# xswang/xflow

Measured on NVIDIA H100. Metric: training examples/sec, higher is better.
Workload: dtype f32

## Files before the change

### xflow_b200/csrc/kernels.cu

```cuda
#include <cuda_runtime.h>
#include <stdint.h>
#include <stdlib.h>

#include "kernels.h"
#include "table.cuh"

__global__ void xf_k_fill(uint8_t* base, uint64_t cap, uint32_t stride, int lazy) {
  const uint64_t chunks_per_row = stride / 16;
  const uint64_t total = cap * chunks_per_row;
  for (uint64_t c = (uint64_t)blockIdx.x * blockDim.x + threadIdx.x; c < total;
       c += (uint64_t)gridDim.x * blockDim.x) {
    uint64_t r = c / chunks_per_row;
    uint32_t q = (uint32_t)(c % chunks_per_row);
    uint4 v = make_uint4(0, 0, 0, 0);
    if (q == 0) {
      v.x = 0xFFFFFFFFu; v.y = 0xFFFFFFFFu;
      if (!lazy) v.w = XF_NEG_ZERO_BITS;
    }
    *reinterpret_cast<uint4*>(base + r * stride + (uint64_t)q * 16) = v;
  }
}

template <int VEC>
__device__ __forceinline__ void xf_ldv(const float* p, float (&o)[VEC]) {
  if (VEC == 4) { float4 t = __ldcg(reinterpret_cast<const float4*>(p)); o[0] = t.x; o[1 % VEC] = t.y; o[2 % VEC] = t.z; o[3 % VEC] = t.w; }
  else if (VEC == 2) { float2 t = __ldcg(reinterpret_cast<const float2*>(p)); o[0] = t.x; o[1 % VEC] = t.y; }
  else { o[0] = __ldcg(p); }
}
template <int VEC>
__device__ __forceinline__ void xf_stv(float* p, const float (&o)[VEC]) {
  if (VEC == 4) *reinterpret_cast<float4*>(p) = make_float4(o[0], o[1 % VEC], o[2 % VEC], o[3 % VEC]);
  else if (VEC == 2) *reinterpret_cast<float2*>(p) = make_float2(o[0], o[1 % VEC]);
  else *p = o[0];
}
template <int VEC, bool SLOTG, bool STAMP>
__global__ void __launch_bounds__(256)
xf_k_update(XfTableView t, const uint32_t* __restrict__ slots, uint64_t n, int tps, double rows,
            const float* __restrict__ gw, const float* __restrict__ gv, int part,
            unsigned long long* __restrict__ live_total, const uint32_t* __restrict__ n_dev,
            const uint32_t* __restrict__ rows_dev, uint32_t extra_base, uint32_t extra_n,
            const float* __restrict__ v0_side, XfStampView sv) {
  __shared__ unsigned int s_live;
  if (threadIdx.x == 0) s_live = 0;
  __syncthreads();
  uint64_t n_head = n;
  if (n_dev != nullptr) {
    n_head = min((uint64_t)__ldg(n_dev), (uint64_t)extra_base);
    n = n_head + extra_n;
    rows = (double)__ldg(rows_dev);
  }
  unsigned int live_acc = 0;
  const int K = t.K;
  const unsigned lane = threadIdx.x & 31u;
  const uint64_t gwarp = ((uint64_t)blockIdx.x * blockDim.x + threadIdx.x) >> 5;
  const uint64_t nwarps = ((uint64_t)gridDim.x * blockDim.x) >> 5;
  const int q = (int)(lane & (unsigned)(tps - 1));
  const int gi = (int)(lane / (unsigned)tps);
  const int ngroups = 32 / tps;
  const int leader = (int)(lane & ~(unsigned)(tps - 1));
  const unsigned group_mask = (tps == 32) ? 0xffffffffu : (((1u << tps) - 1u) << leader);
  const int nchunk = K / VEC;

  for (uint64_t base = gwarp * 32; base < n; base += nwarps * 32) {
    const uint64_t e_fwd = base + lane;
    const uint64_t e_i = (SLOTG && e_fwd < n) ? (n - 1 - e_fwd) : e_fwd;
    const uint64_t e_phys = (e_i < n_head) ? e_i : (uint64_t)extra_base + (e_i - n_head);
    const uint32_t s_lane = (e_fwd < n) ? __ldcs(slots + e_phys) : 0xFFFFFFFFu;
    unsigned pend = __ballot_sync(0xffffffffu, s_lane != 0xFFFFFFFFu);
    if (live_total != nullptr && lane == 0) live_acc += __popc(pend);

    while (pend) {
      const int cnt = __popc(pend);
      const unsigned src = (gi < cnt) ? __fns(pend, 0, gi + 1) : 0u;
      const uint32_t s = __shfl_sync(0xffffffffu, s_lane, (int)src);
      const uint64_t i = __shfl_sync(0xffffffffu, (unsigned long long)e_i, (int)src);
      const uint64_t i_phys = __shfl_sync(0xffffffffu, (unsigned long long)e_phys, (int)src);
      uint8_t* rowp = (gi < cnt) ? xf_row(t, s) : nullptr;
      pend = (cnt <= ngroups) ? 0u : (pend & ~((2u << __fns(pend, 0, ngroups)) - 1u));

      const bool lat = K > 0 && (part & 2) && rowp != nullptr;
      float* vp = lat ? xf_row_v(rowp) : nullptr;
      float* nvp = lat ? xf_row_nv(rowp, K) : nullptr;
      float* zvp = lat ? xf_row_zv(rowp, K) : nullptr;
      float v0[VEC], n0[VEC], z0[VEC];
#pragma unroll
      for (int e = 0; e < VEC; ++e) { v0[e] = 0.f; n0[e] = 0.f; z0[e] = 0.f; }
      const bool has0 = lat && q < nchunk;
      if (has0) {
        xf_ldv<VEC>(vp + q * VEC, v0);
        if (t.opt == XF_OPT_FTRL) { xf_ldv<VEC>(nvp + q * VEC, n0); xf_ldv<VEC>(zvp + q * VEC, z0); }
      }
      float p0[VEC];
#pragma unroll
      for (int e = 0; e < VEC; ++e) p0[e] = 0.f;
      if (SLOTG && v0_side != nullptr && has0) {
        const uint64_t tok = (i_phys < (uint64_t)extra_base) ? i_phys : (uint64_t)__ldg(slots + i_phys + extra_n);
        xf_ldv<VEC>(v0_side + tok * (uint64_t)K + q * VEC, p0);
      }
      float ca0[VEC];
#pragma unroll
      for (int e = 0; e < VEC; ++e) ca0[e] = 0.f;
      if (SLOTG && t.canon && has0) xf_ldv<VEC>(xf_row_ca(t, rowp) + q * VEC, ca0);
      double accL = 0.0, accA = 0.0;
      if (SLOTG && has0) {
        const double2 a = __ldcg(reinterpret_cast<const double2*>(xf_row_acc(rowp, K)));
        accL = a.x;
        accA = a.y;
      }
      XfHead h;
      h.key = 0; h.flags = 0; h.w = h.n = h.z = 0.f; h.g = 0.0;
      if (q == 0 && rowp != nullptr) h = xf_load_head(rowp);
      const uint64_t key = __shfl_sync(group_mask, (unsigned long long)h.key, leader);
      const uint32_t flags = __shfl_sync(group_mask, h.flags, leader);
      if (rowp == nullptr) continue;

      if (q == 0) {
        if (!SLOTG) xf_apply_pending(t, h);
        if (part & 1) {
          const float g = SLOTG ? xf_div_rows((float)h.g, rows) : gw[i];
          xf_opt_coord(t, g, h.w, h.n, h.z);
        }
        if (SLOTG) h.g = -0.0;
        if (K > 0 && (part & 2)) h.flags |= XF_FLAG_V_READY;
        xf_store_head_t(t, rowp, h);
        if (STAMP) sv.stamp[s] = sv.now;
      }
      if (lat) {
        const bool ready = (flags & XF_FLAG_V_READY) != 0;
        for (int c = q; c < nchunk; c += tps) {
          const int k = c * VEC;
          float v[VEC], g[VEC], nn[VEC], zz[VEC];
#pragma unroll
          for (int e = 0; e < VEC; ++e) { v[e] = v0[e]; nn[e] = n0[e]; zz[e] = z0[e]; }
          if (c != q && ready) {
            xf_ldv<VEC>(vp + k, v);
            if (t.opt == XF_OPT_FTRL) { xf_ldv<VEC>(nvp + k, nn); xf_ldv<VEC>(zvp + k, zz); }
          }
          if (!ready) {
#pragma unroll
            for (int e = 0; e < VEC; ++e) { v[e] = xf_v_init(t, key, (uint32_t)(k + e)); nn[e] = 0.f; zz[e] = 0.f; }
          }
          if (SLOTG) {
            float vp0[VEC];
#pragma unroll
            for (int e = 0; e < VEC; ++e) vp0[e] = v[e];
            if (v0_side != nullptr) {
              if (c == q) {
#pragma unroll
                for (int e = 0; e < VEC; ++e) vp0[e] = p0[e];
              } else {
                const uint64_t tok = (i_phys < (uint64_t)extra_base) ? i_phys : (uint64_t)__ldg(slots + i_phys + extra_n);
                xf_ldv<VEC>(v0_side + tok * (uint64_t)K + k, vp0);
              }
            }
            if (t.canon) {
              float ca[VEC];
#pragma unroll
              for (int e = 0; e < VEC; ++e) ca[e] = ca0[e];
              if (c != q) xf_ldv<VEC>(xf_row_ca(t, rowp) + k, ca);
#pragma unroll
              for (int e = 0; e < VEC; ++e) g[e] = xf_div_rows((float)((double)ca[e] - (double)vp0[e] * accL), rows);
              const float zero[VEC] = {};
              xf_stv<VEC>(xf_row_ca(t, rowp) + k, zero);
            } else {
#pragma unroll
              for (int e = 0; e < VEC; ++e) g[e] = xf_div_rows((float)(accA - (double)vp0[e] * accL), rows);
            }
          } else {
#pragma unroll
            for (int e = 0; e < VEC; ++e) g[e] = gv[i * (uint64_t)K + k + e];
          }
          if (t.opt == XF_OPT_FTRL) {
#pragma unroll
            for (int e = 0; e < VEC; ++e) xf_ftrl_coord(t, g[e], v[e], nn[e], zz[e]);
            xf_stv<VEC>(nvp + k, nn);
            xf_stv<VEC>(zvp + k, zz);
          } else {
#pragma unroll
            for (int e = 0; e < VEC; ++e) xf_sgd_coord(t, g[e], v[e]);
          }
          xf_stv<VEC>(vp + k, v);
        }
        if (SLOTG) {
          __syncwarp(group_mask);
          if (q == 0) *reinterpret_cast<double2*>(xf_row_acc(rowp, K)) = make_double2(0.0, 0.0);
        }
      }
    }
  }
  if (live_total != nullptr) {
    if (lane == 0 && live_acc) atomicAdd(&s_live, live_acc);
    __syncthreads();
    if (threadIdx.x == 0 && s_live) atomicAdd_system(live_total, (unsigned long long)s_live);
  }
}

template <bool INSERT>
__global__ void xf_k_probe(XfTableView t, const uint64_t* __restrict__ keys, uint64_t n,
                           uint32_t* __restrict__ slots, float* __restrict__ w_out, XfStampView sv) {
  for (uint64_t i = (uint64_t)blockIdx.x * blockDim.x + threadIdx.x; i < n;
       i += (uint64_t)gridDim.x * blockDim.x) {
    XfHead h;
    h.w = 0.f;
    int64_t s = xf_probe<INSERT, true>(t, keys[i], &h, &sv);
    slots[i] = s >= 0 ? (uint32_t)s : 0xFFFFFFFFu;
    if (w_out) {
      if (s >= 0) xf_apply_pending(t, h);
      w_out[i] = s >= 0 ? h.w : 0.f;
    }
  }
}

__global__ void xf_k_gather_v(XfTableView t, const uint32_t* __restrict__ slots, const uint64_t* __restrict__ keys,
                              uint64_t n, float* __restrict__ v_out) {
  const int K = t.K;
  const uint64_t total = n * (uint64_t)K;
  for (uint64_t x = (uint64_t)blockIdx.x * blockDim.x + threadIdx.x; x < total;
       x += (uint64_t)gridDim.x * blockDim.x) {
    const uint64_t i = x / K;
    const int k = (int)(x % K);
    const uint32_t s = slots[i];
    float v = 0.f;
    if (s != 0xFFFFFFFFu) {
      const uint8_t* rowp = xf_row(t, s);
      const uint32_t flags = __ldcg(reinterpret_cast<const uint32_t*>(rowp + XF_OFF_FLAGS));
      v = (flags & XF_FLAG_V_READY) ? __ldcg(reinterpret_cast<const float*>(rowp + 32) + k)
                                    : xf_v_init(t, keys[i], (uint32_t)k);
    }
    v_out[x] = v;
  }
}

__global__ void xf_k_import(XfTableView t, const uint32_t* __restrict__ slots, uint64_t n,
                            const float* w, const float* nw, const float* zw, const float* v,
                            const float* nv, const float* zv) {
  const int K = t.K;
  const uint64_t per = (uint64_t)K + 1;
  const uint64_t total = n * per;
  for (uint64_t x = (uint64_t)blockIdx.x * blockDim.x + threadIdx.x; x < total;
       x += (uint64_t)gridDim.x * blockDim.x) {
    const uint64_t i = x / per;
    const int c = (int)(x % per);
    const uint32_t s = slots[i];
    if (s == 0xFFFFFFFFu) continue;
    uint8_t* rowp = xf_row(t, s);
    if (c == 0) {
      if (w) {
        if (t.lazy) {
          XfHead h;
          h.key = *reinterpret_cast<const uint64_t*>(rowp);
          h.w = w[i]; h.n = nw ? nw[i] : 0.f; h.z = zw ? zw[i] : 0.f; h.flags = 0u; h.g = 0.0;
          xf_lazy_store(t, rowp, h, true);
        } else {
          *reinterpret_cast<float2*>(rowp + XF_OFF_STATE) = make_float2(w[i], nw ? nw[i] : 0.f);
          *reinterpret_cast<float*>(rowp + XF_OFF_STATE + 8) = zw ? zw[i] : 0.f;
          *reinterpret_cast<unsigned long long*>(rowp + 8) = XF_NEG_ZERO_BITS64;
        }
      }
      if (v && K > 0) *reinterpret_cast<uint32_t*>(rowp + XF_OFF_FLAGS) = XF_FLAG_V_READY;
    } else if (v) {
      const int k = c - 1;
      xf_row_v(rowp)[k] = v[i * K + k];
      if (k == 0) *reinterpret_cast<double2*>(xf_row_acc(rowp, K)) = make_double2(0.0, 0.0);
      if (t.opt == XF_OPT_FTRL) {
        xf_row_nv(rowp, K)[k] = nv ? nv[i * K + k] : 0.f;
        xf_row_zv(rowp, K)[k] = zv ? zv[i * K + k] : 0.f;
      }
    }
  }
}

__global__ void xf_k_export(XfTableView t, const uint32_t* __restrict__ slots, const uint64_t* __restrict__ keys,
                            uint64_t n, float* w, float* nw, float* zw, float* v, float* nv, float* zv,
                            uint8_t* present) {
  const int K = t.K;
  const uint64_t per = (uint64_t)K + 1;
  const uint64_t total = n * per;
  for (uint64_t x = (uint64_t)blockIdx.x * blockDim.x + threadIdx.x; x < total;
       x += (uint64_t)gridDim.x * blockDim.x) {
    const uint64_t i = x / per;
    const int c = (int)(x % per);
    const uint32_t s = slots[i];
    const bool have = s != 0xFFFFFFFFu;
    const uint8_t* rowp = have ? xf_row(t, s) : nullptr;
    if (c == 0) {
      XfHead h;
      h.w = h.n = h.z = 0.f;
      if (have) {
        h = xf_load_head(rowp);
        xf_apply_pending(t, h);
      }
      if (present) present[i] = have ? 1 : 0;
      if (w) w[i] = h.w;
      if (nw) nw[i] = h.n;
      if (zw) zw[i] = h.z;
    } else if (v) {
      const int k = c - 1;
      float vv = 0.f, nn = 0.f, zz = 0.f;
      if (have) {
        const uint32_t flags = __ldcg(reinterpret_cast<const uint32_t*>(rowp + XF_OFF_FLAGS));
        if (flags & XF_FLAG_V_READY) {
          vv = __ldcg(reinterpret_cast<const float*>(rowp + 32) + k);
          if (t.opt == XF_OPT_FTRL) {
            nn = __ldcg(xf_row_nv(const_cast<uint8_t*>(rowp), K) + k);
            zz = __ldcg(xf_row_zv(const_cast<uint8_t*>(rowp), K) + k);
          }
        } else {
          vv = xf_v_init(t, keys[i], (uint32_t)k);
        }
      }
      v[i * K + k] = vv;
      if (nv) nv[i * K + k] = nn;
      if (zv) zv[i * K + k] = zz;
    }
  }
}

__global__ void xf_k_rehash(XfTableView src, XfTableView dst, XfKeep keep, const uint32_t* __restrict__ src_stamp,
                            uint32_t* __restrict__ dst_stamp) {
  const uint64_t cap = src.mask + 1;
  const uint32_t chunks = src.stride / 16;
  for (uint64_t r = (uint64_t)blockIdx.x * blockDim.x + threadIdx.x; r < cap;
       r += (uint64_t)gridDim.x * blockDim.x) {
    const uint8_t* srow = xf_row(src, r);
    uint4 a = *reinterpret_cast<const uint4*>(srow);
    uint64_t key = (uint64_t)a.x | ((uint64_t)a.y << 32);
    if (key == XF_EMPTY_KEY) continue;
    const uint32_t stamp = src_stamp != nullptr ? src_stamp[r] : 0u;
    if (src_stamp != nullptr && !xf_keeps(keep, stamp, key)) continue;
    XfHead h;
    int64_t s = xf_probe<true>(dst, key, &h);
    if (s < 0) continue;
    uint8_t* drow = xf_row(dst, (uint64_t)s);
    *reinterpret_cast<uint2*>(drow + 8) = make_uint2(a.z, a.w);
    for (uint32_t c = 1; c < chunks; ++c)
      *reinterpret_cast<uint4*>(drow + 16 * c) = *reinterpret_cast<const uint4*>(srow + 16 * c);
    if (dst_stamp != nullptr) dst_stamp[s] = stamp;
  }
}

__global__ void xf_k_list_keys(XfTableView t, uint64_t* keys_out, unsigned long long* count, uint64_t max_out) {
  const uint64_t cap = t.mask + 1;
  for (uint64_t r = (uint64_t)blockIdx.x * blockDim.x + threadIdx.x; r < cap;
       r += (uint64_t)gridDim.x * blockDim.x) {
    const uint64_t key = *reinterpret_cast<const uint64_t*>(xf_row(t, r));
    if (key == XF_EMPTY_KEY) continue;
    unsigned long long idx = atomicAdd(count, 1ull);
    if (idx < max_out) keys_out[idx] = key;
  }
}

static int g_sm_count = 0;
int xf_sms() {
  if (g_sm_count == 0) {
    int dev = 0;
    cudaGetDevice(&dev);
    cudaDeviceGetAttribute(&g_sm_count, cudaDevAttrMultiProcessorCount, dev);
    if (g_sm_count <= 0) g_sm_count = 132;
  }
  return g_sm_count;
}
int xf_grid_for(uint64_t work_items, int block, int blocks_per_sm) {
  uint64_t want = (work_items + block - 1) / block;
  uint64_t cap = (uint64_t)xf_sms() * blocks_per_sm;
  if (want < 1) want = 1;
  return (int)(want < cap ? want : cap);
}

int xf_vec_for(int K) { return K <= 0 ? 1 : (K % 4 == 0 ? 4 : (K % 2 == 0 ? 2 : 1)); }
int xf_tps_for(int K) {
  if (K <= 0) return 1;
  int chunks = K / xf_vec_for(K);
  int tps = 1;
  while (tps < chunks && tps < 32) tps <<= 1;
  return tps;
}

void xf_launch_fill(const XfTableView& t, cudaStream_t st) {
  uint64_t cap = t.mask + 1;
  uint64_t total = cap * (t.stride / 16);
  xf_k_fill<<<xf_grid_for(total, 256, 16), 256, 0, st>>>(t.base, cap, t.stride, t.lazy);
}

template <bool SLOTG, bool STAMP = false>
static void xf_launch_update_t(const XfTableView& t, const uint32_t* slots, uint64_t n, double rows,
                               const float* gw, const float* gv, int part, unsigned long long* live_total,
                               cudaStream_t st, const uint32_t* n_dev = nullptr, const uint32_t* rows_dev = nullptr,
                               uint32_t extra_base = 0, uint32_t extra_n = 0, const float* v0_side = nullptr,
                               XfStampView sv = XfStampView{nullptr, 0u}) {
  const int tps = xf_tps_for(t.K);
  const int grid = xf_grid_for(n * (uint64_t)tps, 256, 8);
#define XF_UPD_ARGS t, slots, n, tps, rows, gw, gv, part, live_total, n_dev, rows_dev, extra_base, extra_n, v0_side, sv
  switch (xf_vec_for(t.K)) {
    case 4: xf_k_update<4, SLOTG, STAMP><<<grid, 256, 0, st>>>(XF_UPD_ARGS); break;
    case 2: xf_k_update<2, SLOTG, STAMP><<<grid, 256, 0, st>>>(XF_UPD_ARGS); break;
    default: xf_k_update<1, SLOTG, STAMP><<<grid, 256, 0, st>>>(XF_UPD_ARGS); break;
  }
#undef XF_UPD_ARGS
}

void xf_launch_update_touched_dev(const XfTableView& t, const uint32_t* touched, uint64_t work_bound,
                                  const uint32_t* n_dev, const uint32_t* rows_dev, uint32_t extra_base,
                                  uint32_t extra_n, const float* v0_side, unsigned long long* unique_total,
                                  cudaStream_t st) {
  xf_launch_update_t<true>(t, touched, work_bound + extra_n, 1.0, nullptr, nullptr, 3, unique_total, st, n_dev, rows_dev,
                           extra_base, extra_n, v0_side);
}

__global__ void xf_k_flush_pending(XfTableView t) {
  const uint64_t cap = t.mask + 1;
  for (uint64_t r = (uint64_t)blockIdx.x * blockDim.x + threadIdx.x; r < cap; r += (uint64_t)gridDim.x * blockDim.x) {
    uint8_t* rowp = xf_row(t, r);
    XfHead h = xf_load_head(rowp);
    if (h.key == XF_EMPTY_KEY || !xf_lazy_has_pending(h)) continue;
    xf_apply_pending(t, h);
    xf_lazy_store(t, rowp, h);
  }
}
void xf_launch_flush_pending(const XfTableView& t, cudaStream_t st) {
  xf_k_flush_pending<<<xf_grid_for(t.mask + 1, 256, 8), 256, 0, st>>>(t);
}

void xf_launch_update_touched(const XfTableView& t, const uint32_t* touched, uint64_t nnz, double rows,
                              unsigned long long* unique_total, const XfStampView& sv, cudaStream_t st) {
  if (nnz == 0) return;
  if (sv.stamp)
    xf_launch_update_t<true, true>(t, touched, nnz, rows, nullptr, nullptr, 3, unique_total, st, nullptr, nullptr, 0, 0,
                                   nullptr, sv);
  else
    xf_launch_update_t<true>(t, touched, nnz, rows, nullptr, nullptr, 3, unique_total, st);
}

void xf_launch_update_pushed(const XfTableView& t, const uint32_t* slots, uint64_t n, const float* gw,
                             const float* gv, cudaStream_t st) {
  if (n == 0) return;
  int part = (gw ? 1 : 0) | (gv ? 2 : 0);
  xf_launch_update_t<false>(t, slots, n, 1.0, gw, gv, part, nullptr, st);
}

void xf_launch_probe(const XfTableView& t, const uint64_t* keys, uint64_t n, bool insert, uint32_t* slots,
                     float* w_out, cudaStream_t st, const XfStampView& sv) {
  if (n == 0) return;
  const int grid = xf_grid_for(n, 256, 8);
  if (insert) xf_k_probe<true><<<grid, 256, 0, st>>>(t, keys, n, slots, w_out, sv);
  else xf_k_probe<false><<<grid, 256, 0, st>>>(t, keys, n, slots, w_out, sv);
}

void xf_launch_gather_v(const XfTableView& t, const uint32_t* slots, const uint64_t* keys, uint64_t n,
                        float* v_out, cudaStream_t st) {
  if (n == 0 || t.K == 0) return;
  xf_k_gather_v<<<xf_grid_for(n * t.K, 256, 8), 256, 0, st>>>(t, slots, keys, n, v_out);
}

void xf_launch_import(const XfTableView& t, const uint32_t* slots, uint64_t n, const float* w, const float* nw,
                      const float* zw, const float* v, const float* nv, const float* zv, cudaStream_t st) {
  if (n == 0) return;
  xf_k_import<<<xf_grid_for(n * (t.K + 1), 256, 8), 256, 0, st>>>(t, slots, n, w, nw, zw, v, nv, zv);
}

void xf_launch_export(const XfTableView& t, const uint32_t* slots, const uint64_t* keys, uint64_t n, float* w,
                      float* nw, float* zw, float* v, float* nv, float* zv, uint8_t* present, cudaStream_t st) {
  if (n == 0) return;
  xf_k_export<<<xf_grid_for(n * (t.K + 1), 256, 8), 256, 0, st>>>(t, slots, keys, n, w, nw, zw, v, nv, zv, present);
}

void xf_launch_rehash(const XfTableView& src, const XfTableView& dst, const XfKeep& keep, const uint32_t* src_stamp,
                      uint32_t* dst_stamp, cudaStream_t st) {
  xf_k_rehash<<<xf_grid_for(src.mask + 1, 256, 8), 256, 0, st>>>(src, dst, keep, src_stamp, dst_stamp);
}

void xf_launch_list_keys(const XfTableView& t, uint64_t* keys_out, unsigned long long* count, uint64_t max_out,
                         cudaStream_t st) {
  xf_k_list_keys<<<xf_grid_for(t.mask + 1, 256, 8), 256, 0, st>>>(t, keys_out, count, max_out);
}
```

### xflow_b200/csrc/mg_kernels.cu

```cuda
#include <cuda_runtime.h>
#include <stdint.h>

#include "kernels.h"
#include "mg.cuh"
#include "table.cuh"

#define XF_NO_SLOT 0xFFFFFFFFu

__device__ __forceinline__ unsigned long long xf_globaltimer() {
  unsigned long long t;
  asm volatile("mov.u64 %0, %%globaltimer;" : "=l"(t));
  return t;
}
__device__ __forceinline__ uint64_t xf_ld_acquire_sys(const uint64_t* p) {
  uint64_t v;
  asm volatile("ld.acquire.sys.global.u64 %0, [%1];" : "=l"(v) : "l"(p) : "memory");
  return v;
}
__device__ __forceinline__ void xf_st_release_sys(uint64_t* p, uint64_t v) {
  asm volatile("st.release.sys.global.u64 [%0], %1;" ::"l"(p), "l"(v) : "memory");
}

__global__ void xf_k_signal(XfPeers peers, XfSlabLayout L, int S, int me, int flag, uint64_t step, int parity,
                            const uint32_t* __restrict__ bucket_cnt, uint32_t rows) {
  const int q = threadIdx.x;
  if (q >= S) return;
  uint8_t* slab = peers.slab[q];
  if (bucket_cnt != nullptr) {
    volatile uint32_t* m = reinterpret_cast<uint32_t*>(slab + L.off_meta) + ((size_t)(parity * XF_MG_MAX_SHARDS + me) * 4);
    m[0] = bucket_cnt[q];
    m[1] = rows;
  }
  xf_st_release_sys(reinterpret_cast<uint64_t*>(slab + L.off_flags) + (size_t)flag * XF_MG_MAX_SHARDS + me, step);
}

__global__ void xf_k_wait(const uint64_t* __restrict__ flags, int S, uint64_t step, int* error,
                          unsigned long long timeout_ns) {
  const int q = threadIdx.x;
  if (q >= S) return;
  const unsigned long long t0 = xf_globaltimer();
  while (xf_ld_acquire_sys(flags + q) < step) {
    if (xf_globaltimer() - t0 > timeout_ns) {
      *error = 4;
      break;
    }
    __nanosleep(64);
  }
}

#define XF_RT_THREADS 512
#define XF_RT_TOK 4
#define XF_RT_TILE (XF_RT_THREADS * XF_RT_TOK)

__device__ __forceinline__ int xf_dev_shard_of(uint64_t key, uint64_t width, int S) {
  const uint64_t s = key / width;
  return (int)(s < (uint64_t)S ? s : (uint64_t)S - 1);
}

__device__ __forceinline__ uint32_t xf_row_of(const uint32_t* a, uint32_t lo, uint32_t hi, uint32_t j) {
  while (lo < hi) {
    const uint32_t mid = (lo + hi + 1) >> 1;
    if (a[mid] <= j) lo = mid; else hi = mid - 1;
  }
  return lo;
}

__global__ void __launch_bounds__(XF_RT_THREADS)
xf_k_route(const uint32_t* __restrict__ row_ptr, const uint64_t* __restrict__ keys, uint32_t rows, uint64_t width,
           int S, int me, uint32_t cap, XfPeers peers, uint64_t off_keys, uint64_t off_rows,
           uint32_t* __restrict__ bucket_cnt, uint32_t* __restrict__ tok_pos) {
  __shared__ uint64_t s_key[XF_RT_TILE];
  __shared__ uint32_t s_row[XF_RT_TILE];
  __shared__ uint32_t s_rp[XF_RT_TILE + 1];
  __shared__ uint32_t s_cnt[XF_MG_MAX_SHARDS], s_base[XF_MG_MAX_SHARDS], s_off[XF_MG_MAX_SHARDS + 1];
  __shared__ uint32_t s_rlo, s_rhi;
  const uint32_t beg = __ldg(row_ptr), end = __ldg(row_ptr + rows);
  const uint32_t j0 = beg + blockIdx.x * XF_RT_TILE;
  if (j0 >= end) return;
  const uint32_t j1 = min(j0 + (uint32_t)XF_RT_TILE, end);
  if (threadIdx.x < XF_MG_MAX_SHARDS) s_cnt[threadIdx.x] = 0;
  if (threadIdx.x == 0) s_rlo = xf_row_of(row_ptr, 0, rows - 1, j0);
  if (threadIdx.x == 32) s_rhi = xf_row_of(row_ptr, 0, rows - 1, j1 - 1);
  __syncthreads();
  const uint32_t rlo = s_rlo, rhi = s_rhi;
  const bool cached = (rhi - rlo + 1) <= (uint32_t)XF_RT_TILE;
  if (cached)
    for (uint32_t r = threadIdx.x; r <= rhi - rlo + 1; r += XF_RT_THREADS) s_rp[r] = __ldg(row_ptr + rlo + r);
  __syncthreads();

  uint64_t my_key[XF_RT_TOK];
  uint32_t my_rank[XF_RT_TOK], my_row[XF_RT_TOK];
  int my_q[XF_RT_TOK];
#pragma unroll
  for (int i = 0; i < XF_RT_TOK; ++i) {
    const uint32_t j = j0 + threadIdx.x + i * XF_RT_THREADS;
    my_q[i] = -1;
    if (j < j1) {
      my_key[i] = __ldcs(keys + j);
      my_q[i] = xf_dev_shard_of(my_key[i], width, S);
      my_rank[i] = atomicAdd(&s_cnt[my_q[i]], 1u);
      my_row[i] = cached ? (rlo + xf_row_of(s_rp, 0, rhi - rlo, j)) : xf_row_of(row_ptr, rlo, rhi, j);
    }
  }
  __syncthreads();
  if (threadIdx.x < S && s_cnt[threadIdx.x]) s_base[threadIdx.x] = atomicAdd(bucket_cnt + threadIdx.x, s_cnt[threadIdx.x]);
  if (threadIdx.x == 0) {
    uint32_t o = 0;
    for (int q = 0; q < S; ++q) { s_off[q] = o; o += s_cnt[q]; }
    s_off[S] = o;
  }
  __syncthreads();
#pragma unroll
  for (int i = 0; i < XF_RT_TOK; ++i) {
    if (my_q[i] < 0) continue;
    const uint32_t j = j0 + threadIdx.x + i * XF_RT_THREADS;
    const uint32_t at = s_off[my_q[i]] + my_rank[i];
    s_key[at] = my_key[i];
    s_row[at] = my_row[i];
    tok_pos[j] = (uint32_t)my_q[i] * cap + s_base[my_q[i]] + my_rank[i];
  }
  __syncthreads();
  const uint32_t n = j1 - j0;
  for (uint32_t x = threadIdx.x; x < n; x += XF_RT_THREADS) {
    int q = 0;
    while (x >= s_off[q + 1]) ++q;
    const uint64_t dst = (uint64_t)me * cap + s_base[q] + (x - s_off[q]);
    reinterpret_cast<uint64_t*>(peers.slab[q] + off_keys)[dst] = s_key[x];
    reinterpret_cast<uint32_t*>(peers.slab[q] + off_rows)[dst] = s_row[x];
  }
}

template <bool FM, int VEC>
__global__ void __launch_bounds__(256)
xf_k_pull_tokens(XfTableView t, const uint64_t* __restrict__ in_keys, const uint32_t* __restrict__ meta, int S, int me,
                 uint32_t cap, XfPeers peers, uint64_t off_vals, uint32_t* __restrict__ slots,
                 float* __restrict__ side_v, uint4* __restrict__ stash) {
  __shared__ uint32_t s_pre[XF_MG_MAX_SHARDS + 1];
  if (threadIdx.x == 0) {
    uint32_t o = 0;
    for (int s = 0; s < S; ++s) { s_pre[s] = o; o += min(meta[s * 4], cap); }
    s_pre[S] = o;
  }
  __syncthreads();
  const uint32_t total = s_pre[S];
  const int K = t.K;
  for (uint32_t x = blockIdx.x * blockDim.x + threadIdx.x; x < total; x += gridDim.x * blockDim.x) {
    int s = 0;
    while (x >= s_pre[s + 1]) ++s;
    const uint32_t i = x - s_pre[s];
    const uint64_t key = __ldcs(in_keys + (uint64_t)s * cap + i);
    const uint64_t home = xf_home_slot(t, key);
    XfHead h = FM ? xf_load_head_l1(xf_row(t, home)) : xf_load_head(xf_row(t, home));
    const int64_t r = xf_probe_from<true>(t, key, home, h);
    float w = 0.f, st = 0.f, qt = 0.f;
    if (!FM && stash != nullptr) {
      const uint64_t q1 = xf_raw_q1(h), q2 = xf_raw_q2(h);
      uint64_t q3 = xf_raw_q3(h);
      if ((uint32_t)(q1 >> 32) == xf_lazy_check(q2)) q3 |= XF_TAG_MASK;
      __stcs(stash + ((uint64_t)s * cap + i), make_uint4((uint32_t)q2, (uint32_t)(q2 >> 32), (uint32_t)q3, (uint32_t)(q3 >> 32)));
    }
    if (r >= 0) {
      xf_apply_pending(t, h);
      w = h.w;
      if (FM) {
        float* sv = (s > 0 && side_v != nullptr) ? side_v + ((uint64_t)s * cap + i) * (uint64_t)K : nullptr;
        if ((h.flags & XF_FLAG_V_READY) && (K & 7) == 0) {
          const float* vp = reinterpret_cast<const float*>(xf_row(t, (uint64_t)r) + 32);
          for (int k = 0; k < K; k += 8) {
            float v[8];
            xf_ld8_l1(vp + k, v);
#pragma unroll
            for (int e = 0; e < 8; ++e) { st += v[e]; qt = __fadd_rn(qt, __fmul_rn(v[e], v[e])); }
            if (sv) {
              __stcs(reinterpret_cast<float4*>(sv + k), make_float4(v[0], v[1], v[2], v[3]));
              __stcs(reinterpret_cast<float4*>(sv + k + 4), make_float4(v[4], v[5], v[6], v[7]));
            }
          }
        } else if (h.flags & XF_FLAG_V_READY) {
          const float* vp = reinterpret_cast<const float*>(xf_row(t, (uint64_t)r) + 32);
          for (int k = 0; k < K; k += VEC) {
            float v[VEC];
            if (VEC == 4) { const float4 q4 = __ldca(reinterpret_cast<const float4*>(vp + k)); v[0] = q4.x; v[1 % VEC] = q4.y; v[2 % VEC] = q4.z; v[3 % VEC] = q4.w; }
            else if (VEC == 2) { const float2 q2 = __ldca(reinterpret_cast<const float2*>(vp + k)); v[0] = q2.x; v[1 % VEC] = q2.y; }
            else { v[0] = __ldca(vp + k); }
#pragma unroll
            for (int e = 0; e < VEC; ++e) { st += v[e]; qt = __fadd_rn(qt, __fmul_rn(v[e], v[e])); }
            if (sv) {
              if (VEC == 4) __stcs(reinterpret_cast<float4*>(sv + k), make_float4(v[0], v[1 % VEC], v[2 % VEC], v[3 % VEC]));
              else if (VEC == 2) __stcs(reinterpret_cast<float2*>(sv + k), make_float2(v[0], v[1 % VEC]));
              else __stcs(sv + k, v[0]);
            }
          }
        } else {
          for (int k = 0; k < K; ++k) {
            const float v = xf_v_init(t, key, (uint32_t)k);
            st += v;
            qt = __fadd_rn(qt, __fmul_rn(v, v));
            if (sv) __stcs(sv + k, v);
          }
        }
      }
    }
    slots[(uint64_t)s * cap + i] = r >= 0 ? (uint32_t)r : XF_NO_SLOT;
    const uint64_t dst = (uint64_t)me * cap + i;
    if (FM) reinterpret_cast<float4*>(peers.slab[s] + off_vals)[dst] = make_float4(w, st, qt, 0.f);
    else reinterpret_cast<float*>(peers.slab[s] + off_vals)[dst] = w;
  }
}

template <bool FM>
__global__ void __launch_bounds__(256)
xf_k_rows(const uint32_t* __restrict__ row_ptr, const uint8_t* __restrict__ labels, int B, int mode,
          const uint32_t* __restrict__ tok_pos, const void* __restrict__ vals, float* __restrict__ rowv,
          float* __restrict__ loss_out, float* __restrict__ pctr_out, float* __restrict__ abs_loss_sum) {
  __shared__ float s_abs[8];
  float abs_acc = 0.f;
  const int lane = threadIdx.x & 31;
  const int wpb = blockDim.x >> 5;
  const int gwarp = blockIdx.x * wpb + (threadIdx.x >> 5);
  const int nwarps = gridDim.x * wpb;
  for (int row = gwarp; row < B; row += nwarps) {
    const uint32_t beg = __ldg(row_ptr + row), end = __ldg(row_ptr + row + 1);
    float wsum = 0.f, ssum = 0.f, qsum = 0.f;
    for (uint32_t j = beg + lane; j < end; j += 32) {
      const uint32_t pos = __ldcs(tok_pos + j);
      if (FM) {
        const float4 a = __ldcg(reinterpret_cast<const float4*>(vals) + pos);
        wsum += a.x; ssum += a.y; qsum += a.z;
      } else {
        wsum += __ldcg(reinterpret_cast<const float*>(vals) + pos);
      }
    }
    const float wx = xf_warp_sum(wsum);
    float Ssum = 0.f, arg = wx;
    if (FM) {
      Ssum = xf_warp_sum(ssum);
      const float Q = xf_warp_sum(qsum);
      arg = __fadd_rn(wx, __fsub_rn(__fmul_rn(Ssum, Ssum), Q));
    }
    const float pctr = xf_sigmoid(arg);
    if (mode == 1) {
      if (lane == 0 && pctr_out) pctr_out[row] = pctr;
      continue;
    }
    const float loss = __fsub_rn(pctr, (float)labels[row]);
    if (lane == 0) {
      if (loss_out) loss_out[row] = loss;
      if (FM) reinterpret_cast<float2*>(rowv)[row] = make_float2(loss, Ssum);
      else rowv[row] = loss;
    }
    abs_acc += fabsf(loss);
  }
  if (abs_loss_sum != nullptr && mode == 0) {
    if (lane == 0) s_abs[threadIdx.x >> 5] = abs_acc;
    __syncthreads();
    if (threadIdx.x == 0) {
      float tot = 0.f;
      for (int w = 0; w < wpb; ++w) tot += s_abs[w];
      atomicAdd(abs_loss_sum, tot);
    }
  }
}

__global__ void xf_k_bcast_rowv(const uint32_t* __restrict__ src, uint32_t n_words, XfPeers peers, uint64_t off_rowv,
                                uint64_t dst_word_off) {
  uint32_t* dst = reinterpret_cast<uint32_t*>(peers.slab[blockIdx.y] + off_rowv) + dst_word_off;
  for (uint32_t x = blockIdx.x * blockDim.x + threadIdx.x; x < n_words; x += gridDim.x * blockDim.x) dst[x] = __ldcg(src + x);
}

__global__ void __launch_bounds__(256)
xf_k_push_tokens_lr(XfTableView t, const uint32_t* __restrict__ slots, const uint32_t* __restrict__ in_rows,
                    const float* __restrict__ rowv, const uint32_t* __restrict__ meta_s, uint32_t cap, uint32_t seq,
                    uint64_t* rows_by_seq, unsigned long long* uniq_remote, const uint4* __restrict__ stash) {
  __shared__ unsigned int s_open;
  if (threadIdx.x == 0) s_open = 0;
  const uint32_t n = min(__ldg(meta_s), cap);
  const int fs = xf_fix_shift(n);
  if (blockIdx.x == 0 && threadIdx.x == 0)
    rows_by_seq[seq] = (uint64_t)__ldg(meta_s + 1) | ((uint64_t)fs << 32);
  __syncthreads();
  unsigned int open_acc = 0;
  const int lane = threadIdx.x & 31;
  const uint32_t wpb = blockDim.x >> 5;
  const uint32_t gwarp = blockIdx.x * wpb + (threadIdx.x >> 5);
  const uint32_t nwarps = gridDim.x * wpb;
  uint32_t s_n[2], r_n[2];
  uint4 b_n[2];
#define XF_PUSH_FETCH(base_)                                                        \
  _Pragma("unroll") for (int u = 0; u < 2; ++u) {                                    \
    const uint32_t i = (base_) + 32u * u + lane;                                     \
    s_n[u] = XF_NO_SLOT; r_n[u] = 0u; b_n[u] = make_uint4(0u, 0u, 0u, 0u);            \
    if (i < n) {                                                                     \
      s_n[u] = __ldcs(slots + i);                                                    \
      r_n[u] = __ldcs(in_rows + i);                                                  \
      b_n[u] = __ldcs(stash + (uint64_t)i);                                          \
    }                                                                                \
  }
  uint32_t base = gwarp * 64;
  if (base < n) { XF_PUSH_FETCH(base) }
  for (; base < n; base += nwarps * 64) {
    uint32_t s[2];
    float l[2];
    uint64_t q2[2], q3[2];
#pragma unroll
    for (int u = 0; u < 2; ++u) {
      s[u] = s_n[u];
      l[u] = 0.f;
      q2[u] = 0ull; q3[u] = (uint64_t)seq;
      if (s[u] == XF_NO_SLOT) continue;
      l[u] = __ldcg(rowv + r_n[u]);
      q2[u] = (uint64_t)b_n[u].x | ((uint64_t)b_n[u].y << 32);
      q3[u] = (uint64_t)b_n[u].z | ((uint64_t)b_n[u].w << 32);
    }
    if (base + nwarps * 64 < n) { XF_PUSH_FETCH(base + nwarps * 64) }
    bool lead[2], issued[2], reload[2];
    long long fix[2];
    uint64_t q2n[2], o2[2], o3[2];
#pragma unroll
    for (int u = 0; u < 2; ++u) {
      const bool valid = s[u] != XF_NO_SLOT;
      const unsigned grp = __match_any_sync(0xffffffffu, valid ? s[u] : (0xFFFFFF00u | (uint32_t)lane));
      lead[u] = valid && lane == __ffs(grp) - 1;
      fix[u] = valid ? xf_fix_of(l[u], fs) : 0ll;
      if (__any_sync(0xffffffffu, valid && __popc(grp) > 1)) {
        long long sum = 0ll;
        for (int b = 0; b < 32; ++b) {
          const long long o = __shfl_sync(0xffffffffu, fix[u], b);
          if ((grp >> b) & 1u) sum += o;
        }
        fix[u] = sum;
      }
      issued[u] = false;
      q2n[u] = q2[u]; o2[u] = q2[u]; o3[u] = q3[u];
      reload[u] = lead[u] && (q3[u] & XF_TAG_MASK) == XF_TAG_MASK;
      if (lead[u] && !reload[u]) {
        xf_lazy_fold(t, 0ull, q2[u], q3[u], seq, q2n[u]);
        issued[u] = xf_lazy_deposit_issue(xf_row(t, s[u]), q2[u], q3[u], q2n[u], seq, fix[u], o2[u], o3[u]);
      }
    }
#pragma unroll
    for (int u = 0; u < 2; ++u) {
      if (!lead[u]) continue;
      uint8_t* rowp = xf_row(t, s[u]);
      bool stale = false;
      if (!reload[u] &&
          xf_lazy_deposit_resolve(rowp, issued[u], q2[u], q3[u], o2[u], o3[u], seq, fix[u], &stale))
        ++open_acc;
      if (stale) {
        uint64_t r2n;
        xf_lazy_fold(t, 0ull, o2[u], o3[u], seq, r2n);
        if (xf_lazy_deposit(t, rowp, o2[u], o3[u], r2n, seq, fix[u])) ++open_acc;
      } else if (reload[u]) {
        const XfHead h = xf_load_head(rowp);
        uint64_t r2n;
        xf_lazy_fold(t, xf_raw_q1(h), xf_raw_q2(h), xf_raw_q3(h), seq, r2n);
        if (xf_lazy_deposit(t, rowp, xf_raw_q2(h), xf_raw_q3(h), r2n, seq, fix[u])) ++open_acc;
      }
    }
  }
#undef XF_PUSH_FETCH
  if (open_acc) atomicAdd(&s_open, open_acc);
  __syncthreads();
  if (threadIdx.x == 0 && s_open && uniq_remote) atomicAdd_system(uniq_remote, (unsigned long long)s_open);
}

template <bool FM>
__global__ void __launch_bounds__(256)
xf_k_acc_tokens(XfTableView t, const uint32_t* __restrict__ slots, const uint32_t* __restrict__ in_rows,
                const void* __restrict__ rowv, const uint32_t* __restrict__ meta_s, uint32_t cap,
                uint32_t* __restrict__ touched, int log2nc) {
  extern __shared__ __align__(16) unsigned char xf_smem[];
  const int K = t.K;
  const int NC = (FM && log2nc >= 0) ? (1 << log2nc) : 0;
  double* c_acc = reinterpret_cast<double*>(xf_smem);
  uint32_t* c_tag = reinterpret_cast<uint32_t*>(xf_smem + (size_t)NC * 24);
  uint32_t* c_tok = c_tag + NC;
  if (NC) {
    for (int e = threadIdx.x; e < NC; e += blockDim.x) { c_tag[e] = XF_NO_SLOT; c_tok[e] = 0; }
    for (int e = threadIdx.x; e < NC * 3; e += blockDim.x) c_acc[e] = 0.0;
    __syncthreads();
  }
  const uint32_t n = min(__ldg(meta_s), cap);
  const int lane = threadIdx.x & 31;
  const uint32_t wpb = blockDim.x >> 5;
  const uint32_t gwarp = blockIdx.x * wpb + (threadIdx.x >> 5);
  const uint32_t nwarps = gridDim.x * wpb;
  for (uint32_t base = gwarp * 32; base < n; base += nwarps * 32) {
    const uint32_t i = base + lane;
    uint32_t s = XF_NO_SLOT;
    float loss = 0.f, Srow = 0.f;
    if (i < n) {
      s = __ldcs(slots + i);
      const uint32_t row = __ldcs(in_rows + i);
      if (FM) { const float2 a = __ldcg(reinterpret_cast<const float2*>(rowv) + row); loss = a.x; Srow = a.y; }
      else loss = __ldcg(reinterpret_cast<const float*>(rowv) + row);
    }
    const bool valid = s != XF_NO_SLOT;
    float gw_c = loss;
    if (FM) {
      gw_c = 0.f;
      for (int k = 0; k < K; ++k) gw_c += loss;
    }
    double gd = (double)gw_c, ld = (double)loss, ad = (double)loss * (double)Srow;
    const unsigned grp = __match_any_sync(0xffffffffu, valid ? s : (0xFFFFFF00u | (uint32_t)lane));
    const bool lead = valid && lane == __ffs(grp) - 1;
    if (__any_sync(0xffffffffu, valid && __popc(grp) > 1)) {
      double sg = 0.0, sl = 0.0, sa = 0.0;
      for (int b = 0; b < 32; ++b) {
        const double og = __shfl_sync(0xffffffffu, gd, b), ol = __shfl_sync(0xffffffffu, ld, b),
                     oa = __shfl_sync(0xffffffffu, ad, b);
        if ((grp >> b) & 1u) { sg += og; sl += ol; sa += oa; }
      }
      gd = sg; ld = sl; ad = sa;
    }
    bool first = false;
    if (lead) {
      bool cached = false;
      if (NC) {
        const uint32_t e = (s * 2654435761u) >> (32 - log2nc);
        const uint32_t prev = atomicCAS(c_tag + e, XF_NO_SLOT, s);
        if (prev == XF_NO_SLOT || prev == s) {
          cached = true;
          if (prev == XF_NO_SLOT) c_tok[e] = i;
          atomicAdd(c_acc + 3 * e, gd);
          atomicAdd(c_acc + 3 * e + 1, ld);
          atomicAdd(c_acc + 3 * e + 2, ad);
        }
      }
      if (!cached) {
        uint8_t* rowp = xf_row(t, s);
        const double old = atomicAdd(xf_row_g(rowp), gd);
        if (FM) { double* a = xf_row_acc(rowp, K); atomicAdd(a, ld); atomicAdd(a + 1, ad); }
        first = (unsigned long long)__double_as_longlong(old) == XF_NEG_ZERO_BITS64;
      }
    }
    if (i < n) __stcs(touched + i, first ? s : XF_NO_SLOT);
  }
  if (NC) {
    __syncthreads();
    for (int e = threadIdx.x; e < NC; e += blockDim.x) {
      const uint32_t s = c_tag[e];
      uint32_t rec = XF_NO_SLOT;
      if (s != XF_NO_SLOT) {
        uint8_t* rowp = xf_row(t, s);
        const double old = atomicAdd(xf_row_g(rowp), c_acc[3 * e]);
        if ((unsigned long long)__double_as_longlong(old) == XF_NEG_ZERO_BITS64) rec = s;
        double* a = xf_row_acc(rowp, K);
        atomicAdd(a, c_acc[3 * e + 1]);
        atomicAdd(a + 1, c_acc[3 * e + 2]);
      }
      touched[cap + (uint32_t)blockIdx.x * (uint32_t)NC + (uint32_t)e] = rec;
      touched[cap + (gridDim.x + (uint32_t)blockIdx.x) * (uint32_t)NC + (uint32_t)e] = c_tok[e];
    }
  }
}

int xf_step_cache_log2(int K);

void xf_launch_signal(const XfPeers& peers, const XfSlabLayout& L, int S, int me, int flag, uint64_t step, int parity,
                      const uint32_t* bucket_cnt, uint32_t rows, cudaStream_t st) {
  xf_k_signal<<<1, 32, 0, st>>>(peers, L, S, me, flag, step, parity, bucket_cnt, rows);
}
void xf_launch_wait(const uint64_t* flags, int S, uint64_t step, int* error, unsigned long long timeout_ns,
                    cudaStream_t st) {
  xf_k_wait<<<1, 32, 0, st>>>(flags, S, step, error, timeout_ns);
}
void xf_launch_route(const uint32_t* row_ptr, const uint64_t* keys, uint32_t rows, uint32_t nnz_bound, uint64_t width,
                     int S, int me, uint32_t cap, const XfPeers& peers, uint64_t off_keys, uint64_t off_rows,
                     uint32_t* bucket_cnt, uint32_t* tok_pos, cudaStream_t st) {
  if (rows == 0 || nnz_bound == 0) return;
  const uint32_t grid = (nnz_bound + XF_RT_TILE - 1) / XF_RT_TILE;
  xf_k_route<<<grid, XF_RT_THREADS, 0, st>>>(row_ptr, keys, rows, width, S, me, cap, peers, off_keys, off_rows,
                                              bucket_cnt, tok_pos);
}
void xf_launch_pull_tokens(const XfTableView& t, const uint64_t* in_keys, const uint32_t* meta, int S, int me,
                           uint32_t cap, uint64_t work_bound, const XfPeers& peers, uint64_t off_vals,
                           uint32_t* slots, float* side_v, void* stash, cudaStream_t st) {
  const int grid = xf_grid_for(work_bound ? work_bound : 1, 256, 8);
#define XF_PT_ARGS t, in_keys, meta, S, me, cap, peers, off_vals, slots, side_v, reinterpret_cast<uint4*>(stash)
  if (t.K == 0) {
    xf_k_pull_tokens<false, 1><<<grid, 256, 0, st>>>(XF_PT_ARGS);
  } else {
    switch (xf_vec_for(t.K)) {
      case 4: xf_k_pull_tokens<true, 4><<<grid, 256, 0, st>>>(XF_PT_ARGS); break;
      case 2: xf_k_pull_tokens<true, 2><<<grid, 256, 0, st>>>(XF_PT_ARGS); break;
      default: xf_k_pull_tokens<true, 1><<<grid, 256, 0, st>>>(XF_PT_ARGS); break;
    }
  }
#undef XF_PT_ARGS
}
void xf_launch_rows(bool fm, const uint32_t* row_ptr, const uint8_t* labels, int B, int mode, const uint32_t* tok_pos,
                    const void* vals, float* rowv, float* loss_out, float* pctr_out, float* abs_loss_sum,
                    cudaStream_t st) {
  if (B <= 0) return;
  const int grid = xf_grid_for((uint64_t)B * 32, 256, 8);
  if (fm) xf_k_rows<true><<<grid, 256, 0, st>>>(row_ptr, labels, B, mode, tok_pos, vals, rowv, loss_out, pctr_out, abs_loss_sum);
  else xf_k_rows<false><<<grid, 256, 0, st>>>(row_ptr, labels, B, mode, tok_pos, vals, rowv, loss_out, pctr_out, abs_loss_sum);
}
void xf_launch_bcast_rowv(const float* src, uint32_t n_words, int S, const XfPeers& peers, uint64_t off_rowv,
                          uint64_t dst_word_off, cudaStream_t st) {
  if (n_words == 0) return;
  dim3 grid((unsigned)xf_grid_for(n_words, 256, 1), (unsigned)S);
  if (grid.x > 64) grid.x = 64;
  xf_k_bcast_rowv<<<grid, 256, 0, st>>>(reinterpret_cast<const uint32_t*>(src), n_words, peers, off_rowv, dst_word_off);
}
void xf_launch_push_tokens_lr(const XfTableView& t, const uint32_t* slots, const uint32_t* in_rows, const float* rowv,
                              const uint32_t* meta_s, uint32_t cap, uint64_t work_bound, uint32_t seq,
                              uint64_t* rows_by_seq, unsigned long long* uniq_remote, const void* stash,
                              cudaStream_t st) {
  const int grid = xf_grid_for(work_bound ? work_bound : 1, 256, 8);
  xf_k_push_tokens_lr<<<grid, 256, 0, st>>>(t, slots, in_rows, rowv, meta_s, cap, seq, rows_by_seq, uniq_remote,
                                             reinterpret_cast<const uint4*>(stash));
}
uint32_t xf_acc_touched_extra(int K, uint64_t work_bound) {
  const int lg = xf_step_cache_log2(K);
  if (lg < 0) return 0;
  return (uint32_t)xf_grid_for(work_bound ? work_bound : 1, 256, 8) << lg;
}
void xf_launch_acc_tokens(const XfTableView& t, const uint32_t* slots, const uint32_t* in_rows, const void* rowv,
                          const uint32_t* meta_s, uint32_t cap, uint64_t work_bound, uint32_t* touched,
                          cudaStream_t st) {
  const int grid = xf_grid_for(work_bound ? work_bound : 1, 256, 8);
  const int lg = xf_step_cache_log2(t.K);
  const size_t smem = lg >= 0 ? ((size_t)1 << lg) * 32 : 0;
  if (t.K > 0) xf_k_acc_tokens<true><<<grid, 256, smem, st>>>(t, slots, in_rows, rowv, meta_s, cap, touched, lg);
  else xf_k_acc_tokens<false><<<grid, 256, 0, st>>>(t, slots, in_rows, rowv, meta_s, cap, touched, -1);
}
```

### xflow_b200/csrc/step.cu

```cuda
#include <cuda_runtime.h>
#include <stdint.h>
#include <stdlib.h>

#include "kernels.h"
#include "table.cuh"

#define XF_NO_SLOT 0xFFFFFFFFu
#define XF_CACHED_CHUNKS 2

template <int VEC>
__device__ __forceinline__ void xf_ldv_step(const float* p, float (&o)[VEC]) {
  if (VEC == 4) { float4 t = __ldca(reinterpret_cast<const float4*>(p)); o[0] = t.x; o[1 % VEC] = t.y; o[2 % VEC] = t.z; o[3 % VEC] = t.w; }
  else if (VEC == 2) { float2 t = __ldca(reinterpret_cast<const float2*>(p)); o[0] = t.x; o[1 % VEC] = t.y; }
  else { o[0] = __ldca(p); }
}
template <int VEC>
__device__ __forceinline__ void xf_fm_token(const XfTableView& t, uint32_t slot, uint32_t flags, uint64_t key,
                                            float& st, float& qt) {
  const int K = t.K;
  st = 0.f;
  qt = 0.f;
  if ((flags & XF_FLAG_V_READY) && (K & 7) == 0) {
    const float* vp = reinterpret_cast<const float*>(xf_row(t, slot) + 32);
    for (int k = 0; k < K; k += 8) {
      float v[8];
      xf_ld8_l1(vp + k, v);
#pragma unroll
      for (int e = 0; e < 8; ++e) { st += v[e]; qt = __fadd_rn(qt, __fmul_rn(v[e], v[e])); }
    }
  } else if (flags & XF_FLAG_V_READY) {
    const float* vp = reinterpret_cast<const float*>(xf_row(t, slot) + 32);
    for (int k = 0; k < K; k += VEC) {
      float v[VEC];
      xf_ldv_step<VEC>(vp + k, v);
#pragma unroll
      for (int e = 0; e < VEC; ++e) { st += v[e]; qt = __fadd_rn(qt, __fmul_rn(v[e], v[e])); }
    }
  } else {
    for (int k = 0; k < K; ++k) {
      const float v = xf_v_init(t, key, (uint32_t)k);
      st += v;
      qt = __fadd_rn(qt, __fmul_rn(v, v));
    }
  }
}

template <bool FM, int VEC, bool ADMIT, bool STAMP, bool WEIGHT>
__global__ void __launch_bounds__(256)
xf_k_step(XfTableView t, const uint32_t* __restrict__ row_ptr, const uint64_t* __restrict__ keys,
          const uint8_t* __restrict__ labels, int B, int mode, uint32_t* __restrict__ touched,
          float* __restrict__ loss_out, float* __restrict__ pctr_out, float* __restrict__ abs_loss_sum,
          int log2nc, uint32_t touched_base, XfAdmitView adm, XfStampView sv, XfWeightView wv) {
  __shared__ float s_abs[8];
  extern __shared__ __align__(16) unsigned char xf_smem[];
  float abs_acc = 0.f;
  const int lane = threadIdx.x & 31;
  const int warps_per_block = blockDim.x >> 5;
  const int gwarp = blockIdx.x * warps_per_block + (threadIdx.x >> 5);
  const int nwarps = gridDim.x * warps_per_block;
  const int K = t.K;
  const int NC = (FM && log2nc >= 0) ? (1 << log2nc) : 0;
  double* c_acc = reinterpret_cast<double*>(xf_smem);
  uint32_t* c_tag = reinterpret_cast<uint32_t*>(xf_smem + (size_t)NC * 24);
  if (NC) {
    for (int e = threadIdx.x; e < NC; e += blockDim.x) c_tag[e] = XF_NO_SLOT;
    for (int e = threadIdx.x; e < NC * 3; e += blockDim.x) c_acc[e] = 0.0;
    __syncthreads();
  }

  for (int row = gwarp; row < B; row += nwarps) {
    const uint32_t beg = __ldg(row_ptr + row);
    const uint32_t end = __ldg(row_ptr + row + 1);
    if (WEIGHT && __ldg(wv.e + row) == 0.f) {
      if (lane == 0 && loss_out) loss_out[row] = 0.f;
      for (uint32_t j = beg + (uint32_t)lane; j < end; j += 32u) __stcs(touched + j, XF_NO_SLOT);
      continue;
    }
    const int chunks = (int)((end - beg + 63u) >> 6);

    float wsum = 0.f, ssum = 0.f, qsum = 0.f;
    uint32_t slot_c[2 * XF_CACHED_CHUNKS];
#pragma unroll
    for (int c = 0; c < 2 * XF_CACHED_CHUNKS; ++c) slot_c[c] = XF_NO_SLOT;

    for (int ch = 0; ch < chunks; ++ch) {
      const uint32_t j0 = beg + (uint32_t)ch * 64u + (uint32_t)lane;
      const uint32_t j1 = j0 + 32u;
      const bool v0 = j0 < end, v1 = j1 < end;
      const uint64_t k0 = v0 ? __ldcs(keys + j0) : 0ull;
      const uint64_t k1 = v1 ? __ldcs(keys + j1) : 0ull;
      const uint64_t p0 = xf_home_slot(t, k0), p1 = xf_home_slot(t, k1);
      XfHead h0, h1;
      h0.key = h1.key = XF_EMPTY_KEY;
      if (v0) h0 = FM ? xf_load_head_l1(xf_row(t, p0)) : xf_load_head(xf_row(t, p0));
      if (v1) h1 = FM ? xf_load_head_l1(xf_row(t, p1)) : xf_load_head(xf_row(t, p1));
      uint32_t s0 = XF_NO_SLOT, s1 = XF_NO_SLOT;
      bool r0 = false, r1 = false;
      if (v0) {
        const int64_t r = xf_probe_from<true, ADMIT, STAMP>(t, k0, p0, h0, &adm, &r0, &sv);
        if (r >= 0) { s0 = (uint32_t)r; wsum += h0.w; }
      }
      if (v1) {
        const int64_t r = xf_probe_from<true, ADMIT, STAMP>(t, k1, p1, h1, &adm, &r1, &sv);
        if (r >= 0) { s1 = (uint32_t)r; wsum += h1.w; }
      }
      if (ADMIT) xf_admit_append(adm, r0, k0, r1, k1);
      if (FM) {
        float st, qt;
        if (s0 != XF_NO_SLOT) { xf_fm_token<VEC>(t, s0, h0.flags, k0, st, qt); ssum += st; qsum += qt; }
        if (s1 != XF_NO_SLOT) { xf_fm_token<VEC>(t, s1, h1.flags, k1, st, qt); ssum += st; qsum += qt; }
      }
#pragma unroll
      for (int c = 0; c < XF_CACHED_CHUNKS; ++c)
        if (ch == c) { slot_c[2 * c] = s0; slot_c[2 * c + 1] = s1; }
    }

    const float wx = xf_warp_sum(wsum);
    float S = 0.f, arg = wx;
    if (FM) {
      S = xf_warp_sum(ssum);
      const float Q = xf_warp_sum(qsum);
      const float v_y = __fsub_rn(__fmul_rn(S, S), Q);
      arg = __fadd_rn(wx, v_y);
    }
    const float pctr = xf_sigmoid(arg);
    if (mode == 1) {
      if (lane == 0 && pctr_out) pctr_out[row] = pctr;
      continue;
    }
    float loss = __fsub_rn(pctr, (float)labels[row]);
    if (lane == 0 && loss_out) loss_out[row] = loss;
    if (WEIGHT) loss = __fmul_rn(__ldg(wv.e + row), loss);
    abs_acc += fabsf(loss);

    float gw_c = loss;
    if (FM) {
      gw_c = 0.f;
      for (int k = 0; k < K; ++k) gw_c += loss;
    }
    const double gw_d = (double)gw_c;
    for (int ch = 0; ch < chunks; ++ch) {
      const uint32_t j0 = beg + (uint32_t)ch * 64u + (uint32_t)lane;
      const uint32_t j1 = j0 + 32u;
      uint32_t s0 = XF_NO_SLOT, s1 = XF_NO_SLOT;
      if (ch < XF_CACHED_CHUNKS) {
#pragma unroll
        for (int c = 0; c < XF_CACHED_CHUNKS; ++c)
          if (ch == c) { s0 = slot_c[2 * c]; s1 = slot_c[2 * c + 1]; }
      } else {
        XfHead h;
        if (j0 < end) { const int64_t r = xf_probe<false>(t, __ldg(keys + j0), &h); if (r >= 0) s0 = (uint32_t)r; }
        if (j1 < end) { const int64_t r = xf_probe<false>(t, __ldg(keys + j1), &h); if (r >= 0) s1 = (uint32_t)r; }
      }
      const unsigned g0 = __match_any_sync(0xffffffffu, (s0 != XF_NO_SLOT) ? s0 : (0xFFFFFF00u | (uint32_t)lane));
      const unsigned g1 = __match_any_sync(0xffffffffu, (s1 != XF_NO_SLOT) ? s1 : (0xFFFFFF00u | (uint32_t)lane));
      const bool lead0 = s0 != XF_NO_SLOT && lane == __ffs(g0) - 1;
      const bool lead1 = s1 != XF_NO_SLOT && lane == __ffs(g1) - 1;
      const double c0 = (double)__popc(g0), c1 = (double)__popc(g1);
      const double ld = (double)loss, ad = (double)loss * (double)S;
      double old0 = 0.0, old1 = 0.0;
      bool cached0 = false, cached1 = false;
      if (NC) {
        if (lead0) {
          const uint32_t e = (s0 * 2654435761u) >> (32 - log2nc);
          const uint32_t prev = atomicCAS(c_tag + e, XF_NO_SLOT, s0);
          if (prev == XF_NO_SLOT || prev == s0) {
            cached0 = true;
            atomicAdd(c_acc + 3 * e, gw_d * c0);
            atomicAdd(c_acc + 3 * e + 1, ld * c0);
            atomicAdd(c_acc + 3 * e + 2, ad * c0);
          }
        }
        if (lead1) {
          const uint32_t e = (s1 * 2654435761u) >> (32 - log2nc);
          const uint32_t prev = atomicCAS(c_tag + e, XF_NO_SLOT, s1);
          if (prev == XF_NO_SLOT || prev == s1) {
            cached1 = true;
            atomicAdd(c_acc + 3 * e, gw_d * c1);
            atomicAdd(c_acc + 3 * e + 1, ld * c1);
            atomicAdd(c_acc + 3 * e + 2, ad * c1);
          }
        }
      }
      if (lead0 && !cached0) old0 = atomicAdd(xf_row_g(xf_row(t, s0)), gw_d * c0);
      if (lead1 && !cached1) old1 = atomicAdd(xf_row_g(xf_row(t, s1)), gw_d * c1);
      if (FM) {
        if (lead0 && !cached0) { double* a = xf_row_acc(xf_row(t, s0), K); atomicAdd(a, ld * c0); atomicAdd(a + 1, ad * c0); }
        if (lead1 && !cached1) { double* a = xf_row_acc(xf_row(t, s1), K); atomicAdd(a, ld * c1); atomicAdd(a + 1, ad * c1); }
      }
      const bool f0 = lead0 && !cached0 && (unsigned long long)__double_as_longlong(old0) == XF_NEG_ZERO_BITS64;
      const bool f1 = lead1 && !cached1 && (unsigned long long)__double_as_longlong(old1) == XF_NEG_ZERO_BITS64;
      if (j0 < end) __stcs(touched + j0, f0 ? s0 : XF_NO_SLOT);
      if (j1 < end) __stcs(touched + j1, f1 ? s1 : XF_NO_SLOT);
    }
  }
  if (NC && mode == 0) {
    __syncthreads();
    for (int e = threadIdx.x; e < NC; e += blockDim.x) {
      const uint32_t s = c_tag[e];
      uint32_t rec = XF_NO_SLOT;
      if (s != XF_NO_SLOT) {
        uint8_t* rowp = xf_row(t, s);
        const double old = atomicAdd(xf_row_g(rowp), c_acc[3 * e]);
        if ((unsigned long long)__double_as_longlong(old) == XF_NEG_ZERO_BITS64) rec = s;
        double* a = xf_row_acc(rowp, K);
        atomicAdd(a, c_acc[3 * e + 1]);
        atomicAdd(a + 1, c_acc[3 * e + 2]);
      }
      touched[touched_base + (uint32_t)blockIdx.x * (uint32_t)NC + (uint32_t)e] = rec;
    }
  }
  if (abs_loss_sum != nullptr && mode == 0) {
    if (lane == 0) s_abs[threadIdx.x >> 5] = abs_acc;
    __syncthreads();
    if (threadIdx.x == 0) {
      float tot = 0.f;
      for (int w = 0; w < (int)(blockDim.x >> 5); ++w) tot += s_abs[w];
      atomicAdd(abs_loss_sum, tot);
    }
  }
}

int xf_sms();
int xf_grid_for(uint64_t work_items, int block, int blocks_per_sm);

#define XF_STEP_CACHE_LOG2 9
int xf_step_cache_log2(int K) {
  if (K <= 0) return -1;
  static const int lg = [] {
    const char* e = getenv("XFLOW_FM_CACHE_LOG2");
    const int v = (e && *e) ? atoi(e) : XF_STEP_CACHE_LOG2;
    return v < 0 ? 0 : (v > 10 ? 10 : v);
  }();
  return lg;
}
uint32_t xf_step_touched_extra(int K, int B) {
  const int lg = xf_step_cache_log2(K);
  if (lg < 0) return 0;
  return (uint32_t)xf_grid_for((uint64_t)B * 32, 256, 8) << lg;
}

void xf_launch_step(const XfTableView& t, const uint32_t* row_ptr, const uint64_t* keys, const uint8_t* labels,
                    int B, int mode, uint32_t* touched, uint32_t nnz, float* loss_out, float* pctr_out,
                    float* abs_loss_sum, const XfAdmitView* adm, const XfStampView& sv, const XfWeightView& wv,
                    cudaStream_t st) {
  if (B <= 0) return;
  const int block = 256;
  const int grid = xf_grid_for((uint64_t)B * 32, block, 8);
  const int lg = xf_step_cache_log2(t.K);
  const size_t smem = lg >= 0 ? ((size_t)1 << lg) * 28 : 0;
#define XF_STEP_ARGS t, row_ptr, keys, labels, B, mode, touched, loss_out, pctr_out, abs_loss_sum, lg, nnz, a, sv, wv
#define XF_STEP_LAUNCH_W(A, S, W)                                                             \
  if (t.K == 0) {                                                                             \
    xf_k_step<false, 1, A, S, W><<<grid, block, 0, st>>>(XF_STEP_ARGS);                       \
  } else {                                                                                    \
    switch (xf_vec_for(t.K)) {                                                                \
      case 4: xf_k_step<true, 4, A, S, W><<<grid, block, smem, st>>>(XF_STEP_ARGS); break;    \
      case 2: xf_k_step<true, 2, A, S, W><<<grid, block, smem, st>>>(XF_STEP_ARGS); break;    \
      default: xf_k_step<true, 1, A, S, W><<<grid, block, smem, st>>>(XF_STEP_ARGS); break;   \
    }                                                                                         \
  }
#define XF_STEP_LAUNCH(A, S)        \
  if (wv.e) {                       \
    XF_STEP_LAUNCH_W(A, S, true)    \
  } else {                          \
    XF_STEP_LAUNCH_W(A, S, false)   \
  }
  const XfAdmitView a = adm ? *adm : XfAdmitView{};
  const bool stamp = sv.stamp != nullptr;
  if (adm && stamp) {
    XF_STEP_LAUNCH(true, true)
  } else if (adm) {
    XF_STEP_LAUNCH(true, false)
  } else if (stamp) {
    XF_STEP_LAUNCH(false, true)
  } else {
    XF_STEP_LAUNCH(false, false)
  }
#undef XF_STEP_LAUNCH
#undef XF_STEP_LAUNCH_W
#undef XF_STEP_ARGS
}
```

### xflow_b200/csrc/table.cuh

```cuda
#pragma once
#include <cuda_runtime.h>
#include <stdint.h>

#define XF_EMPTY_KEY 0xFFFFFFFFFFFFFFFFull
#define XF_FLAG_V_READY 1u
#define XF_NEG_ZERO_BITS 0x80000000u
#define XF_NEG_ZERO_BITS64 0x8000000000000000ull
#define XF_MAX_PROBE 8192

enum { XF_OPT_FTRL = 0, XF_OPT_SGD = 1 };
enum { XF_INIT_DEFAULT = 0, XF_INIT_COUNTER = 1, XF_INIT_ZERO = 3 };

struct XfTableView {
  uint8_t* base;
  uint64_t mask;
  uint32_t log2cap;
  uint32_t bshift;
  uint32_t stride;
  int K;
  int opt;
  int v_init;
  float v_const;
  uint64_t seed;
  float alpha, beta, lambda1, lambda2, learning_rate;
  unsigned long long* size;
  int* error;
  int lazy;
  const uint64_t* rows_by_seq;
  int canon;
};
#define XF_ADM_POISSON 1
#define XF_ADM_BLOOM 2
#define XF_ADM_NEVER 3
#define XF_ADM_MAX_HASHES 8
struct XfAdmitView {
  int mode;
  uint32_t p24;
  uint64_t batch_mix;
  uint32_t threshold, log2_cells, hashes;
  uint64_t seed;
  const uint8_t* cells;
  unsigned long long* rej_n;
  uint64_t* rej_keys;
  unsigned long long* admitted;
};
struct XfKeep {
  uint32_t cutoff;
  int bounded;
  uint32_t s_star;
  uint64_t k_star;
};
struct XfStampView {
  uint32_t* stamp;
  uint32_t now;
};
struct XfWeightView {
  const float* e;
  const unsigned long long* W;
};
__host__ __device__ __forceinline__ bool xf_keeps(const XfKeep& k, uint32_t stamp, uint64_t key) {
  return stamp >= k.cutoff && (!k.bounded || stamp > k.s_star || (stamp == k.s_star && key <= k.k_star));
}
#define XF_TAG_LOCKED 0xFFFFFFFFu
#define XF_FIX_MAX_SHIFT 27
#define XF_TAG_MASK 0xFFFFull

__host__ __device__ inline int xf_fix_shift(uint64_t nnz) {
  int bits = 0;
  while (bits < 64 && (nnz >> bits) != 0ull) ++bits;
  const int s = 47 - bits;
  return s > XF_FIX_MAX_SHIFT ? XF_FIX_MAX_SHIFT : (s < 0 ? 0 : s);
}

__host__ __device__ inline uint32_t xf_acc_off(int K) { return (32u + 4u * (uint32_t)K + 15u) & ~15u; }
__host__ __device__ inline uint32_t xf_ca_off(int K, int opt) {
  return xf_acc_off(K) + 16u + ((opt == XF_OPT_FTRL) ? 8u * (uint32_t)K : 0u);
}
__host__ __device__ inline uint32_t xf_row_stride(int K, int opt, int canon = 0) {
  if (K <= 0) return 32u;
  uint32_t bytes = xf_ca_off(K, opt) + (canon ? 4u * (uint32_t)K : 0u);
  return (bytes + 31u) & ~31u;
}

#ifdef __CUDACC__

__device__ __forceinline__ uint64_t xf_probe_slot(const XfTableView& t, uint64_t key, uint32_t i) {
  const uint64_t m = key * 0x9E3779B97F4A7C15ull;
  const uint32_t bs = t.bshift;
  const uint64_t hb = m >> (64 - (t.log2cap - bs));
  const uint32_t b1 = (1u << bs) - 1u;
  const uint32_t j0 = (uint32_t)(m >> 9) & b1;
  const uint32_t k = i >> bs;
  const uint32_t j = (k == 0) ? ((j0 + i) & b1) : (i & b1);
  return (((hb + k) << bs) | j) & t.mask;
}
__device__ __forceinline__ uint64_t xf_home_slot(const XfTableView& t, uint64_t key) { return xf_probe_slot(t, key, 0); }

__host__ __device__ __forceinline__ uint64_t xf_splitmix64(uint64_t x) {
  x += 0x9E3779B97F4A7C15ull;
  x = (x ^ (x >> 30)) * 0xBF58476D1CE4E5B9ull;
  x = (x ^ (x >> 27)) * 0x94D049BB133111EBull;
  return x ^ (x >> 31);
}
__host__ __device__ __forceinline__ uint64_t xf_admit_cell(uint64_t key, uint64_t seed, uint32_t j, uint32_t log2_cells) {
  return xf_splitmix64(key ^ xf_splitmix64(seed + (uint64_t)(j + 1) * 0x9E3779B97F4A7C15ull)) >> (64 - log2_cells);
}
__device__ __forceinline__ bool xf_admit(const XfAdmitView& a, uint64_t key) {
  if (a.mode == XF_ADM_POISSON) return (uint32_t)(xf_splitmix64(key ^ a.batch_mix) >> 40) < a.p24;
  if (a.mode != XF_ADM_BLOOM) return false;
  uint32_t m = 255u;
  for (uint32_t j = 0; j < a.hashes; ++j) m = min(m, (uint32_t)__ldcg(a.cells + xf_admit_cell(key, a.seed, j, a.log2_cells)));
  return m >= a.threshold;
}
__device__ __forceinline__ void xf_admit_append(const XfAdmitView& a, bool r0, uint64_t k0, bool r1, uint64_t k1) {
  const unsigned m0 = __ballot_sync(0xffffffffu, r0), m1 = __ballot_sync(0xffffffffu, r1);
  if ((m0 | m1) == 0u) return;
  const unsigned lane = threadIdx.x & 31u;
  unsigned long long base = 0ull;
  if (lane == 0u) base = atomicAdd(a.rej_n, (unsigned long long)(__popc(m0) + __popc(m1)));
  base = __shfl_sync(0xffffffffu, base, 0);
  if (a.rej_keys) {
    const unsigned lt = (1u << lane) - 1u;
    if (r0) a.rej_keys[base + __popc(m0 & lt)] = k0;
    if (r1) a.rej_keys[base + __popc(m0) + __popc(m1 & lt)] = k1;
  }
}

__device__ __forceinline__ float xf_counter_normal(uint64_t key, uint32_t k, uint64_t seed) {
  uint64_t base = xf_splitmix64(key ^ xf_splitmix64(seed + 0x632BE59BD9B4E019ull * (uint64_t)(k + 1)));
  uint32_t sum = 0;
#pragma unroll
  for (int r = 0; r < 3; ++r) {
    uint64_t x = xf_splitmix64(base + (uint64_t)r);
    sum += (uint32_t)(x & 0xFFFF) + (uint32_t)((x >> 16) & 0xFFFF) + (uint32_t)((x >> 32) & 0xFFFF) +
           (uint32_t)((x >> 48) & 0xFFFF);
  }
  float u = __fmul_rn((float)((int32_t)sum - 6 * 65535), 1.0f / 65536.0f);
  return __fmul_rn(u, 1e-2f);
}
__device__ __forceinline__ float xf_v_init(const XfTableView& t, uint64_t key, uint32_t k) {
  if (t.v_init == XF_INIT_COUNTER) return xf_counter_normal(key, k, t.seed);
  if (t.v_init == XF_INIT_ZERO) return 0.0f;
  return t.v_const;
}

__device__ __forceinline__ uint8_t* xf_row(const XfTableView& t, uint64_t slot) {
  return t.base + slot * (uint64_t)t.stride;
}
__device__ __forceinline__ double* xf_row_g(uint8_t* row) { return reinterpret_cast<double*>(row + 8); }
#define XF_OFF_STATE 16
#define XF_OFF_FLAGS 28
__device__ __forceinline__ float* xf_row_v(uint8_t* row) { return reinterpret_cast<float*>(row + 32); }
__device__ __forceinline__ double* xf_row_acc(uint8_t* row, int K) { return reinterpret_cast<double*>(row + xf_acc_off(K)); }
__device__ __forceinline__ float* xf_row_nv(uint8_t* row, int K) { return reinterpret_cast<float*>(row + xf_acc_off(K) + 16); }
__device__ __forceinline__ float* xf_row_zv(uint8_t* row, int K) { return xf_row_nv(row, K) + K; }
__device__ __forceinline__ float* xf_row_ca(const XfTableView& t, uint8_t* row) { return reinterpret_cast<float*>(row + xf_ca_off(t.K, t.opt)); }

struct XfHead {
  uint64_t key;
  uint32_t flags;
  float w, n, z;
  double g;
};

__device__ __forceinline__ void xf_ld32_cg(const void* p, uint64_t& q0, uint64_t& q1, uint64_t& q2, uint64_t& q3) {
  asm volatile("ld.global.cg.v2.u64 {%0,%1}, [%4];\n\tld.global.cg.v2.u64 {%2,%3}, [%4+16];"
               : "=l"(q0), "=l"(q1), "=l"(q2), "=l"(q3) : "l"(p));
}
__device__ __forceinline__ void xf_ld32_ca(const void* p, uint64_t& q0, uint64_t& q1, uint64_t& q2, uint64_t& q3) {
  asm volatile("ld.global.ca.v2.u64 {%0,%1}, [%4];\n\tld.global.ca.v2.u64 {%2,%3}, [%4+16];"
               : "=l"(q0), "=l"(q1), "=l"(q2), "=l"(q3) : "l"(p));
}
__device__ __forceinline__ void xf_ld32_pair(const uint8_t* mine, uint64_t& q0, uint64_t& q1, uint64_t& q2, uint64_t& q3) {
  const uint32_t odd = threadIdx.x & 1u;
  const uint8_t* other = (const uint8_t*)__shfl_xor_sync(0xffffffffu, (unsigned long long)mine, 1);
  const uint8_t* r0 = odd ? other : mine;
  const uint8_t* r1 = odd ? mine : other;
  uint64_t x0 = 0, x1 = 0, y0 = 0, y1 = 0;
  asm volatile("{\n .reg .pred p0, p1;\n setp.ne.u64 p0, %4, 0;\n setp.ne.u64 p1, %5, 0;\n"
               " @p0 ld.global.cg.v2.u64 {%0,%1}, [%6];\n @p1 ld.global.cg.v2.u64 {%2,%3}, [%7];\n}"
               : "+l"(x0), "+l"(x1), "+l"(y0), "+l"(y1)
               : "l"(r0), "l"(r1), "l"(r0 + 16 * odd), "l"(r1 + 16 * odd));
  const uint64_t m0 = odd ? y0 : x0, m1 = odd ? y1 : x1;
  const uint64_t t0 = __shfl_xor_sync(0xffffffffu, odd ? x0 : y0, 1);
  const uint64_t t1 = __shfl_xor_sync(0xffffffffu, odd ? x1 : y1, 1);
  q0 = odd ? t0 : m0; q1 = odd ? t1 : m1;
  q2 = odd ? m0 : t0; q3 = odd ? m1 : t1;
}
__device__ __forceinline__ void xf_st32(void* p, uint64_t q0, uint64_t q1, uint64_t q2, uint64_t q3) {
  asm volatile("st.global.v2.u64 [%0], {%1,%2};\n\tst.global.v2.u64 [%0+16], {%3,%4};" ::"l"(p), "l"(q0), "l"(q1),
               "l"(q2), "l"(q3)
               : "memory");
}

__device__ __forceinline__ XfHead xf_load_head(const uint8_t* row) {
  uint64_t q0, q1, q2, q3;
  xf_ld32_cg(row, q0, q1, q2, q3);
  XfHead h;
  h.key = q0;
  h.g = __longlong_as_double((long long)q1);
  h.w = __uint_as_float((uint32_t)q2);
  h.n = __uint_as_float((uint32_t)(q2 >> 32));
  h.z = __uint_as_float((uint32_t)q3);
  h.flags = (uint32_t)(q3 >> 32);
  return h;
}

__device__ __forceinline__ XfHead xf_load_head_l1(const uint8_t* row) {
  uint64_t q0, q1, q2, q3;
  xf_ld32_ca(row, q0, q1, q2, q3);
  XfHead h;
  h.key = q0;
  h.g = __longlong_as_double((long long)q1);
  h.w = __uint_as_float((uint32_t)q2);
  h.n = __uint_as_float((uint32_t)(q2 >> 32));
  h.z = __uint_as_float((uint32_t)q3);
  h.flags = (uint32_t)(q3 >> 32);
  return h;
}

__device__ __forceinline__ void xf_ld8_l1(const float* p, float (&o)[8]) {
  uint64_t q0, q1, q2, q3;
  xf_ld32_ca(p, q0, q1, q2, q3);
  o[0] = __uint_as_float((uint32_t)q0); o[1] = __uint_as_float((uint32_t)(q0 >> 32));
  o[2] = __uint_as_float((uint32_t)q1); o[3] = __uint_as_float((uint32_t)(q1 >> 32));
  o[4] = __uint_as_float((uint32_t)q2); o[5] = __uint_as_float((uint32_t)(q2 >> 32));
  o[6] = __uint_as_float((uint32_t)q3); o[7] = __uint_as_float((uint32_t)(q3 >> 32));
}

__device__ __forceinline__ void xf_store_head(uint8_t* row, const XfHead& h) {
  const uint64_t q1 = (uint64_t)__double_as_longlong(h.g);
  const uint64_t q2 = (uint64_t)__float_as_uint(h.w) | ((uint64_t)__float_as_uint(h.n) << 32);
  const uint64_t q3 = (uint64_t)__float_as_uint(h.z) | ((uint64_t)h.flags << 32);
  xf_st32(row, h.key, q1, q2, q3);
}

template <bool INSERT, bool ADMIT = false, bool STAMP = false>
__device__ __forceinline__ int64_t xf_probe_from(const XfTableView& t, uint64_t key, uint64_t s, XfHead& h,
                                                 const XfAdmitView* adm = nullptr, bool* rejected = nullptr,
                                                 const XfStampView* sv = nullptr) {
  for (int probes = 0; probes < XF_MAX_PROBE; ++probes) {
    if (h.key == key) return (int64_t)s;
    if (h.key == XF_EMPTY_KEY) {
      if (!INSERT) return -1;
      if (ADMIT && !xf_admit(*adm, key)) {
        *rejected = adm->mode != XF_ADM_NEVER;
        return -1;
      }
      unsigned long long old =
          atomicCAS(reinterpret_cast<unsigned long long*>(xf_row(t, s)), (unsigned long long)XF_EMPTY_KEY,
                    (unsigned long long)key);
      if (old == XF_EMPTY_KEY) {
        unsigned m = __activemask();
        int leader = __ffs(m) - 1;
        if ((int)(threadIdx.x & 31) == leader) {
          atomicAdd(t.size, (unsigned long long)__popc(m));
          if (ADMIT) atomicAdd(adm->admitted, (unsigned long long)__popc(m));
        }
        if (STAMP && sv->stamp != nullptr) sv->stamp[s] = sv->now;
        h.key = key; h.flags = 0; h.w = 0.f; h.n = 0.f; h.z = 0.f;
        h.g = t.lazy ? 0.0 : -0.0;
        return (int64_t)s;
      }
      if (old == key) {
        h.key = key;
        return (int64_t)s;
      }
    }
    s = xf_probe_slot(t, key, (uint32_t)probes + 1u);
    h = xf_load_head(xf_row(t, s));
  }
  *t.error = 1;
  return -1;
}

template <bool INSERT, bool STAMP = false>
__device__ __forceinline__ int64_t xf_probe(const XfTableView& t, uint64_t key, XfHead* head,
                                            const XfStampView* sv = nullptr) {
  const uint64_t s = xf_home_slot(t, key);
  XfHead h = xf_load_head(xf_row(t, s));
  const int64_t r = xf_probe_from<INSERT, false, STAMP>(t, key, s, h, nullptr, nullptr, sv);
  *head = h;
  return r;
}


__device__ __forceinline__ float xf_sigmoid(float x) {
  if (x < -30.f) return (float)1e-6;
  if (x > 30.f) return 1.0f;
  const double ex = exp((double)x * 0.9999999998311266);
  return (float)(ex / (1.0 + ex));
}

__device__ __forceinline__ void xf_ftrl_coord(const XfTableView& t, float g, float& w, float& n, float& z) {
  float old_n = n;
  float nn = __fadd_rn(old_n, __fmul_rn(g, g));
  float sig = __fdiv_rn(__fsub_rn(__fsqrt_rn(nn), __fsqrt_rn(old_n)), t.alpha);
  z = __fadd_rn(z, __fsub_rn(g, __fmul_rn(sig, w)));
  n = nn;
  if (fabsf(z) <= t.lambda1) {
    w = 0.0f;
  } else {
    float tmpr = 0.0f;
    if (z > 0.0f) tmpr = __fsub_rn(z, t.lambda1);
    if (z < 0.0f) tmpr = __fadd_rn(z, t.lambda1);
    float tmpl = -__fadd_rn(__fdiv_rn(__fadd_rn(t.beta, __fsqrt_rn(n)), t.alpha), t.lambda2);
    w = __fdiv_rn(tmpr, tmpl);
  }
}

__device__ __forceinline__ void xf_sgd_coord(const XfTableView& t, float g, float& w) {
  w = __fsub_rn(w, __fmul_rn(t.learning_rate, g));
}

__device__ __forceinline__ void xf_opt_coord(const XfTableView& t, float g, float& w, float& n, float& z) {
  if (t.opt == XF_OPT_FTRL) xf_ftrl_coord(t, g, w, n, z);
  else xf_sgd_coord(t, g, w);
}

__device__ __forceinline__ float xf_div_rows_plain(float g, double rows) { return (float)((double)g / rows); }
__device__ __forceinline__ float xf_div_rows(float g, double rows) {
  const long long b = __double_as_longlong(rows);
  if ((b & 0x000FFFFFFFFFFFFFll) == 0ll && b > 0ll) {
    const double inv = __longlong_as_double((2046ll << 52) - b);
    return (float)((double)g * inv);
  }
  return (float)((double)g / rows);
}

__device__ __forceinline__ float xf_ftrl_w(const XfTableView& t, float z, float n) {
  if (fabsf(z) <= t.lambda1) return 0.0f;
  float tmpr = 0.0f;
  if (z > 0.0f) tmpr = __fsub_rn(z, t.lambda1);
  if (z < 0.0f) tmpr = __fadd_rn(z, t.lambda1);
  const float tmpl = -__fadd_rn(__fdiv_rn(__fadd_rn(t.beta, __fsqrt_rn(n)), t.alpha), t.lambda2);
  return __fdiv_rn(tmpr, tmpl);
}
__device__ __forceinline__ double xf_pow2(int e) { return __longlong_as_double((long long)(1023 + e) << 52); }
__device__ __forceinline__ long long xf_fix_of(float residual, int shift) {
  return __double2ll_rn((double)residual * xf_pow2(shift));
}

__device__ __forceinline__ uint64_t xf_raw_q2(const XfHead& h) {
  return (uint64_t)__float_as_uint(h.w) | ((uint64_t)__float_as_uint(h.n) << 32);
}
__device__ __forceinline__ uint64_t xf_raw_q3(const XfHead& h) {
  return (uint64_t)__float_as_uint(h.z) | ((uint64_t)h.flags << 32);
}
__device__ __forceinline__ uint64_t xf_raw_q1(const XfHead& h) { return (uint64_t)__double_as_longlong(h.g); }
__device__ __forceinline__ uint32_t xf_lazy_check(uint64_t q2) {
  const uint32_t c = (uint32_t)q2 ^ (uint32_t)(q2 >> 32) ^ 0xA5A5A5A5u;
  return c ? c : 1u;
}
__device__ __forceinline__ float xf_lazy_fold(const XfTableView& t, uint64_t q1, uint64_t q2, uint64_t q3, uint32_t seq,
                                              uint64_t& q2_new) {
  const uint32_t tag = (uint32_t)(q3 & XF_TAG_MASK);
  const bool pending = tag != 0u && tag != seq;
  float g = 0.f;
  if (pending) {
    const long long gfix = (long long)q3 >> 16;
    const uint64_t rs = __ldg(t.rows_by_seq + tag);
    g = xf_div_rows_plain((float)((double)gfix * xf_pow2(-(int)(rs >> 32))), (double)(uint32_t)rs);
  }
  const float a = __uint_as_float((uint32_t)q2), b = __uint_as_float((uint32_t)(q2 >> 32));
  if (t.opt == XF_OPT_FTRL) {
    float n = a, z = b;
    float w = ((uint32_t)(q1 >> 32) == xf_lazy_check(q2)) ? __uint_as_float((uint32_t)q1) : xf_ftrl_w(t, z, n);
    if (pending) xf_ftrl_coord(t, g, w, n, z);
    q2_new = (uint64_t)__float_as_uint(n) | ((uint64_t)__float_as_uint(z) << 32);
    return w;
  }
  float w = a;
  if (pending) xf_sgd_coord(t, g, w);
  q2_new = (uint64_t)__float_as_uint(w);
  return w;
}
__device__ __forceinline__ void xf_apply_pending(const XfTableView& t, XfHead& h) {
  if (!t.lazy) return;
  uint64_t q2n;
  const float w = xf_lazy_fold(t, xf_raw_q1(h), xf_raw_q2(h), xf_raw_q3(h), 0xFFFFFFFFu, q2n);
  h.w = w;
  if (t.opt == XF_OPT_FTRL) {
    h.n = __uint_as_float((uint32_t)q2n);
    h.z = __uint_as_float((uint32_t)(q2n >> 32));
  } else {
    h.n = 0.f;
    h.z = 0.f;
  }
  h.flags = 0u;
  h.g = 0.0;
}
__device__ __forceinline__ bool xf_lazy_has_pending(const XfHead& raw) { return (xf_raw_q3(raw) & XF_TAG_MASK) != 0ull; }
__device__ __forceinline__ void xf_lazy_store(const XfTableView& t, uint8_t* rowp, const XfHead& h, bool keep_w = false) {
  const bool ftrl = t.opt == XF_OPT_FTRL;
  const uint64_t q2 = ftrl ? ((uint64_t)__float_as_uint(h.n) | ((uint64_t)__float_as_uint(h.z) << 32))
                           : (uint64_t)__float_as_uint(h.w);
  uint64_t q1 = 0ull;
  if (keep_w && ftrl && __float_as_uint(h.w) != __float_as_uint(xf_ftrl_w(t, h.z, h.n)))
    q1 = (uint64_t)__float_as_uint(h.w) | ((uint64_t)xf_lazy_check(q2) << 32);
  xf_st32(rowp, h.key, q1, q2, 0ull);
}
__device__ __forceinline__ void xf_store_head_t(const XfTableView& t, uint8_t* rowp, const XfHead& h) {
  if (t.lazy) xf_lazy_store(t, rowp, h);
  else xf_store_head(rowp, h);
}

__device__ __forceinline__ bool xf_cas128(uint8_t* addr, uint64_t e0, uint64_t e1, uint64_t d0, uint64_t d1, uint64_t& o0,
                                          uint64_t& o1) {
  asm volatile(
      "{\n .reg .b128 cmp, swp, old;\n mov.b128 cmp, {%2, %3};\n mov.b128 swp, {%4, %5};\n"
      " atom.global.cas.b128 old, [%6], cmp, swp;\n mov.b128 {%0, %1}, old;\n}"
      : "=l"(o0), "=l"(o1)
      : "l"(e0), "l"(e1), "l"(d0), "l"(d1), "l"(addr)
      : "memory");
  return o0 == e0 && o1 == e1;
}
__device__ __forceinline__ void xf_lazy_add(uint8_t* rowp, long long fix) {
  atomicAdd(reinterpret_cast<unsigned long long*>(rowp + 24), (unsigned long long)fix << 16);
}
__device__ __forceinline__ bool xf_lazy_deposit_issue(uint8_t* rowp, uint64_t q2, uint64_t q3, uint64_t q2_new, uint32_t seq,
                                                      long long fix, uint64_t& o2, uint64_t& o3) {
  if ((uint32_t)(q3 & XF_TAG_MASK) == seq) {
    xf_lazy_add(rowp, fix);
    o2 = q2; o3 = q3;
    return false;
  }
  xf_cas128(rowp + XF_OFF_STATE, q2, q3, q2_new, ((unsigned long long)fix << 16) | (uint64_t)seq, o2, o3);
  return true;
}
__device__ __forceinline__ bool xf_lazy_deposit_resolve(uint8_t* rowp, bool issued, uint64_t q2, uint64_t q3, uint64_t o2,
                                                        uint64_t o3, uint32_t seq, long long fix, bool* stale) {
  *stale = false;
  if (!issued) return false;
  if (o2 == q2 && o3 == q3) return true;
  if ((uint32_t)(o3 & XF_TAG_MASK) == seq) {
    xf_lazy_add(rowp, fix);
    return false;
  }
  *stale = true;
  return false;
}
__device__ __forceinline__ bool xf_lazy_deposit(const XfTableView& t, uint8_t* rowp, uint64_t q2, uint64_t q3, uint64_t q2_new,
                                                uint32_t seq, long long fix, bool* stale = nullptr) {
  if (stale) *stale = false;
  if ((uint32_t)(q3 & XF_TAG_MASK) == seq) {
    xf_lazy_add(rowp, fix);
    return false;
  }
  uint64_t o2, o3;
  if (xf_cas128(rowp + XF_OFF_STATE, q2, q3, q2_new, ((unsigned long long)fix << 16) | (uint64_t)seq, o2, o3)) return true;
  if ((uint32_t)(o3 & XF_TAG_MASK) == seq) {
    xf_lazy_add(rowp, fix);
    return false;
  }
  if (stale) *stale = true;
  else *t.error = 2;
  return false;
}

__device__ __forceinline__ float xf_warp_sum(float v) {
#pragma unroll
  for (int o = 16; o > 0; o >>= 1) v += __shfl_xor_sync(0xffffffffu, v, o);
  return v;
}

#endif
```

Baseline: 83.65 million.

## Cache FM embedding sum and square-sum in row head instead of recomputing

For plain FM tables, the update kernel now computes the per-row sum and sum-of-squares of the latent vector after each update and stores them in the head's gradient word. The step and multi-GPU forward kernels read these two floats from the head rather than loading all K latent values. The scalar weight gradient is folded into the accumulator slot, using K times the loss accumulator, which removes one double atomic per token and shrinks the shared-memory cache. This adds work and an extra shared buffer to the update kernel, and it changes the init and fill layout to match.

```diff
diff --git a/xflow_b200/csrc/kernels.cu b/xflow_b200/csrc/kernels.cu
--- a/xflow_b200/csrc/kernels.cu
+++ b/xflow_b200/csrc/kernels.cu
@@ -5,7 +5,7 @@
 #include "kernels.h"
 #include "table.cuh"
 
-__global__ void xf_k_fill(uint8_t* base, uint64_t cap, uint32_t stride, int lazy) {
+__global__ void xf_k_fill(uint8_t* base, uint64_t cap, uint32_t stride, int lazy, uint32_t l_off) {
   const uint64_t chunks_per_row = stride / 16;
   const uint64_t total = cap * chunks_per_row;
   for (uint64_t c = (uint64_t)blockIdx.x * blockDim.x + threadIdx.x; c < total;
@@ -15,7 +15,9 @@
     uint4 v = make_uint4(0, 0, 0, 0);
     if (q == 0) {
       v.x = 0xFFFFFFFFu; v.y = 0xFFFFFFFFu;
-      if (!lazy) v.w = XF_NEG_ZERO_BITS;
+      if (!lazy && l_off == 0) v.w = XF_NEG_ZERO_BITS;
+    } else if (l_off != 0 && q == l_off / 16) {
+      v.y = XF_NEG_ZERO_BITS;
     }
     *reinterpret_cast<uint4*>(base + r * stride + (uint64_t)q * 16) = v;
   }
@@ -41,6 +43,7 @@
             const uint32_t* __restrict__ rows_dev, uint32_t extra_base, uint32_t extra_n,
             const float* __restrict__ v0_side, XfStampView sv) {
   __shared__ unsigned int s_live;
+  __shared__ float s_vq[256 * VEC];
   if (threadIdx.x == 0) s_live = 0;
   __syncthreads();
   uint64_t n_head = n;
@@ -60,6 +63,7 @@
   const int leader = (int)(lane & ~(unsigned)(tps - 1));
   const unsigned group_mask = (tps == 32) ? 0xffffffffu : (((1u << tps) - 1u) << leader);
   const int nchunk = K / VEC;
+  const bool fm = xf_fm_plain(t);
 
   for (uint64_t base = gwarp * 32; base < n; base += nwarps * 32) {
     const uint64_t e_fwd = base + lane;
@@ -117,12 +121,13 @@
       if (q == 0) {
         if (!SLOTG) xf_apply_pending(t, h);
         if (part & 1) {
-          const float g = SLOTG ? xf_div_rows((float)h.g, rows) : gw[i];
+          const float g = !SLOTG ? gw[i] : fm ? xf_div_rows((float)((double)K * accL), rows) : xf_div_rows((float)h.g, rows);
           xf_opt_coord(t, g, h.w, h.n, h.z);
         }
-        if (SLOTG) h.g = -0.0;
+        if (SLOTG && !fm) h.g = -0.0;
         if (K > 0 && (part & 2)) h.flags |= XF_FLAG_V_READY;
-        xf_store_head_t(t, rowp, h);
+        if (fm && lat) *reinterpret_cast<ulonglong2*>(rowp + XF_OFF_STATE) = make_ulonglong2(xf_raw_q2(h), xf_raw_q3(h));
+        else xf_store_head_t(t, rowp, h);
         if (STAMP) sv.stamp[s] = sv.now;
       }
       if (lat) {
@@ -180,10 +185,33 @@
             for (int e = 0; e < VEC; ++e) xf_sgd_coord(t, g[e], v[e]);
           }
           xf_stv<VEC>(vp + k, v);
+          if (fm && c == q) {
+#pragma unroll
+            for (int e = 0; e < VEC; ++e) s_vq[threadIdx.x * VEC + e] = v[e];
+          }
+        }
+        if (fm) {
+          float S = 0.f, Q = 0.f;
+          __syncwarp(group_mask);
+          if (q == 0) {
+            if (nchunk <= tps) {
+              for (int c = 0; c < nchunk; ++c)
+#pragma unroll
+                for (int e = 0; e < VEC; ++e) xf_fm_sums(s_vq[(threadIdx.x + c) * VEC + e], S, Q);
+            } else {
+              for (int k = 0; k < K; k += VEC) {
+                float x[VEC];
+                xf_ldv<VEC>(vp + k, x);
+#pragma unroll
+                for (int e = 0; e < VEC; ++e) xf_fm_sums(x[e], S, Q);
+              }
+            }
+          }
+          if (q == 0) *reinterpret_cast<ulonglong2*>(rowp) = make_ulonglong2(key, xf_sq_word(S, Q));
         }
         if (SLOTG) {
           __syncwarp(group_mask);
-          if (q == 0) *reinterpret_cast<double2*>(xf_row_acc(rowp, K)) = make_double2(0.0, 0.0);
+          if (q == 0) *reinterpret_cast<double2*>(xf_row_acc(rowp, K)) = make_double2(fm ? -0.0 : 0.0, 0.0);
         }
       }
     }
@@ -235,6 +263,7 @@
                             const float* w, const float* nw, const float* zw, const float* v,
                             const float* nv, const float* zv) {
   const int K = t.K;
+  const bool fm = xf_fm_plain(t);
   const uint64_t per = (uint64_t)K + 1;
   const uint64_t total = n * per;
   for (uint64_t x = (uint64_t)blockIdx.x * blockDim.x + threadIdx.x; x < total;
@@ -254,14 +283,22 @@
         } else {
           *reinterpret_cast<float2*>(rowp + XF_OFF_STATE) = make_float2(w[i], nw ? nw[i] : 0.f);
           *reinterpret_cast<float*>(rowp + XF_OFF_STATE + 8) = zw ? zw[i] : 0.f;
-          *reinterpret_cast<unsigned long long*>(rowp + 8) = XF_NEG_ZERO_BITS64;
+          if (!fm) *reinterpret_cast<unsigned long long*>(rowp + 8) = XF_NEG_ZERO_BITS64;
         }
       }
       if (v && K > 0) *reinterpret_cast<uint32_t*>(rowp + XF_OFF_FLAGS) = XF_FLAG_V_READY;
+      if (fm) {
+        if (v) {
+          float S = 0.f, Q = 0.f;
+          for (int k = 0; k < K; ++k) xf_fm_sums(v[i * K + k], S, Q);
+          *reinterpret_cast<unsigned long long*>(rowp + 8) = xf_sq_word(S, Q);
+        }
+        *reinterpret_cast<double2*>(xf_row_acc(rowp, K)) = make_double2(-0.0, 0.0);
+      }
     } else if (v) {
       const int k = c - 1;
       xf_row_v(rowp)[k] = v[i * K + k];
-      if (k == 0) *reinterpret_cast<double2*>(xf_row_acc(rowp, K)) = make_double2(0.0, 0.0);
+      if (k == 0 && !fm) *reinterpret_cast<double2*>(xf_row_acc(rowp, K)) = make_double2(0.0, 0.0);
       if (t.opt == XF_OPT_FTRL) {
         xf_row_nv(rowp, K)[k] = nv ? nv[i * K + k] : 0.f;
         xf_row_zv(rowp, K)[k] = zv ? zv[i * K + k] : 0.f;
@@ -379,7 +416,8 @@
 void xf_launch_fill(const XfTableView& t, cudaStream_t st) {
   uint64_t cap = t.mask + 1;
   uint64_t total = cap * (t.stride / 16);
-  xf_k_fill<<<xf_grid_for(total, 256, 16), 256, 0, st>>>(t.base, cap, t.stride, t.lazy);
+  const uint32_t l_off = (t.K > 0 && !t.canon) ? xf_acc_off(t.K) : 0u;
+  xf_k_fill<<<xf_grid_for(total, 256, 16), 256, 0, st>>>(t.base, cap, t.stride, t.lazy, l_off);
 }
 
 template <bool SLOTG, bool STAMP = false>
diff --git a/xflow_b200/csrc/mg_kernels.cu b/xflow_b200/csrc/mg_kernels.cu
--- a/xflow_b200/csrc/mg_kernels.cu
+++ b/xflow_b200/csrc/mg_kernels.cu
@@ -164,38 +164,22 @@
       w = h.w;
       if (FM) {
         float* sv = (s > 0 && side_v != nullptr) ? side_v + ((uint64_t)s * cap + i) * (uint64_t)K : nullptr;
-        if ((h.flags & XF_FLAG_V_READY) && (K & 7) == 0) {
-          const float* vp = reinterpret_cast<const float*>(xf_row(t, (uint64_t)r) + 32);
-          for (int k = 0; k < K; k += 8) {
-            float v[8];
-            xf_ld8_l1(vp + k, v);
-#pragma unroll
-            for (int e = 0; e < 8; ++e) { st += v[e]; qt = __fadd_rn(qt, __fmul_rn(v[e], v[e])); }
-            if (sv) {
-              __stcs(reinterpret_cast<float4*>(sv + k), make_float4(v[0], v[1], v[2], v[3]));
-              __stcs(reinterpret_cast<float4*>(sv + k + 4), make_float4(v[4], v[5], v[6], v[7]));
-            }
-          }
-        } else if (h.flags & XF_FLAG_V_READY) {
-          const float* vp = reinterpret_cast<const float*>(xf_row(t, (uint64_t)r) + 32);
-          for (int k = 0; k < K; k += VEC) {
-            float v[VEC];
-            if (VEC == 4) { const float4 q4 = __ldca(reinterpret_cast<const float4*>(vp + k)); v[0] = q4.x; v[1 % VEC] = q4.y; v[2 % VEC] = q4.z; v[3 % VEC] = q4.w; }
-            else if (VEC == 2) { const float2 q2 = __ldca(reinterpret_cast<const float2*>(vp + k)); v[0] = q2.x; v[1 % VEC] = q2.y; }
-            else { v[0] = __ldca(vp + k); }
-#pragma unroll
-            for (int e = 0; e < VEC; ++e) { st += v[e]; qt = __fadd_rn(qt, __fmul_rn(v[e], v[e])); }
-            if (sv) {
-              if (VEC == 4) __stcs(reinterpret_cast<float4*>(sv + k), make_float4(v[0], v[1 % VEC], v[2 % VEC], v[3 % VEC]));
-              else if (VEC == 2) __stcs(reinterpret_cast<float2*>(sv + k), make_float2(v[0], v[1 % VEC]));
-              else __stcs(sv + k, v[0]);
+        if (h.flags & XF_FLAG_V_READY) {
+          const uint64_t sq = (uint64_t)__double_as_longlong(h.g);
+          st = __uint_as_float((uint32_t)sq);
+          qt = __uint_as_float((uint32_t)(sq >> 32));
+          if (sv) {
+            const float* vp = reinterpret_cast<const float*>(xf_row(t, (uint64_t)r) + 32);
+            for (int k = 0; k < K; k += VEC) {
+              if (VEC == 4) __stcs(reinterpret_cast<float4*>(sv + k), __ldca(reinterpret_cast<const float4*>(vp + k)));
+              else if (VEC == 2) __stcs(reinterpret_cast<float2*>(sv + k), __ldca(reinterpret_cast<const float2*>(vp + k)));
+              else __stcs(sv + k, __ldca(vp + k));
             }
           }
         } else {
           for (int k = 0; k < K; ++k) {
             const float v = xf_v_init(t, key, (uint32_t)k);
-            st += v;
-            qt = __fadd_rn(qt, __fmul_rn(v, v));
+            xf_fm_sums(v, st, qt);
             if (sv) __stcs(sv + k, v);
           }
         }
@@ -373,11 +357,11 @@
   const int K = t.K;
   const int NC = (FM && log2nc >= 0) ? (1 << log2nc) : 0;
   double* c_acc = reinterpret_cast<double*>(xf_smem);
-  uint32_t* c_tag = reinterpret_cast<uint32_t*>(xf_smem + (size_t)NC * 24);
+  uint32_t* c_tag = reinterpret_cast<uint32_t*>(xf_smem + (size_t)NC * 16);
   uint32_t* c_tok = c_tag + NC;
   if (NC) {
     for (int e = threadIdx.x; e < NC; e += blockDim.x) { c_tag[e] = XF_NO_SLOT; c_tok[e] = 0; }
-    for (int e = threadIdx.x; e < NC * 3; e += blockDim.x) c_acc[e] = 0.0;
+    for (int e = threadIdx.x; e < NC * 2; e += blockDim.x) c_acc[e] = 0.0;
     __syncthreads();
   }
   const uint32_t n = min(__ldg(meta_s), cap);
@@ -396,12 +380,7 @@
       else loss = __ldcg(reinterpret_cast<const float*>(rowv) + row);
     }
     const bool valid = s != XF_NO_SLOT;
-    float gw_c = loss;
-    if (FM) {
-      gw_c = 0.f;
-      for (int k = 0; k < K; ++k) gw_c += loss;
-    }
-    double gd = (double)gw_c, ld = (double)loss, ad = (double)loss * (double)Srow;
+    double gd = (double)loss, ld = (double)loss, ad = (double)loss * (double)Srow;
     const unsigned grp = __match_any_sync(0xffffffffu, valid ? s : (0xFFFFFF00u | (uint32_t)lane));
     const bool lead = valid && lane == __ffs(grp) - 1;
     if (__any_sync(0xffffffffu, valid && __popc(grp) > 1)) {
@@ -422,15 +401,20 @@
         if (prev == XF_NO_SLOT || prev == s) {
           cached = true;
           if (prev == XF_NO_SLOT) c_tok[e] = i;
-          atomicAdd(c_acc + 3 * e, gd);
-          atomicAdd(c_acc + 3 * e + 1, ld);
-          atomicAdd(c_acc + 3 * e + 2, ad);
+          atomicAdd(c_acc + 2 * e, __dadd_rn(ld, 0.0));
+          atomicAdd(c_acc + 2 * e + 1, ad);
         }
       }
       if (!cached) {
         uint8_t* rowp = xf_row(t, s);
-        const double old = atomicAdd(xf_row_g(rowp), gd);
-        if (FM) { double* a = xf_row_acc(rowp, K); atomicAdd(a, ld); atomicAdd(a + 1, ad); }
+        double old;
+        if (FM) {
+          double* a = xf_row_acc(rowp, K);
+          old = atomicAdd(a, __dadd_rn(ld, 0.0));
+          atomicAdd(a + 1, ad);
+        } else {
+          old = atomicAdd(xf_row_g(rowp), gd);
+        }
         first = (unsigned long long)__double_as_longlong(old) == XF_NEG_ZERO_BITS64;
       }
     }
@@ -442,12 +426,10 @@
       const uint32_t s = c_tag[e];
       uint32_t rec = XF_NO_SLOT;
       if (s != XF_NO_SLOT) {
-        uint8_t* rowp = xf_row(t, s);
-        const double old = atomicAdd(xf_row_g(rowp), c_acc[3 * e]);
+        double* a = xf_row_acc(xf_row(t, s), K);
+        const double old = atomicAdd(a, c_acc[2 * e]);
         if ((unsigned long long)__double_as_longlong(old) == XF_NEG_ZERO_BITS64) rec = s;
-        double* a = xf_row_acc(rowp, K);
-        atomicAdd(a, c_acc[3 * e + 1]);
-        atomicAdd(a + 1, c_acc[3 * e + 2]);
+        atomicAdd(a + 1, c_acc[2 * e + 1]);
       }
       touched[cap + (uint32_t)blockIdx.x * (uint32_t)NC + (uint32_t)e] = rec;
       touched[cap + (gridDim.x + (uint32_t)blockIdx.x) * (uint32_t)NC + (uint32_t)e] = c_tok[e];
@@ -522,7 +504,7 @@
                           cudaStream_t st) {
   const int grid = xf_grid_for(work_bound ? work_bound : 1, 256, 8);
   const int lg = xf_step_cache_log2(t.K);
-  const size_t smem = lg >= 0 ? ((size_t)1 << lg) * 32 : 0;
+  const size_t smem = lg >= 0 ? ((size_t)1 << lg) * 24 : 0;
   if (t.K > 0) xf_k_acc_tokens<true><<<grid, 256, smem, st>>>(t, slots, in_rows, rowv, meta_s, cap, touched, lg);
   else xf_k_acc_tokens<false><<<grid, 256, 0, st>>>(t, slots, in_rows, rowv, meta_s, cap, touched, -1);
 }
diff --git a/xflow_b200/csrc/step.cu b/xflow_b200/csrc/step.cu
--- a/xflow_b200/csrc/step.cu
+++ b/xflow_b200/csrc/step.cu
@@ -8,41 +8,43 @@
 #define XF_NO_SLOT 0xFFFFFFFFu
 #define XF_CACHED_CHUNKS 2
 
-template <int VEC>
-__device__ __forceinline__ void xf_ldv_step(const float* p, float (&o)[VEC]) {
-  if (VEC == 4) { float4 t = __ldca(reinterpret_cast<const float4*>(p)); o[0] = t.x; o[1 % VEC] = t.y; o[2 % VEC] = t.z; o[3 % VEC] = t.w; }
-  else if (VEC == 2) { float2 t = __ldca(reinterpret_cast<const float2*>(p)); o[0] = t.x; o[1 % VEC] = t.y; }
-  else { o[0] = __ldca(p); }
-}
-template <int VEC>
-__device__ __forceinline__ void xf_fm_token(const XfTableView& t, uint32_t slot, uint32_t flags, uint64_t key,
-                                            float& st, float& qt) {
-  const int K = t.K;
+__device__ __forceinline__ void xf_fm_token(const XfTableView& t, uint64_t q1, uint32_t flags, uint64_t key, float& st,
+                                            float& qt) {
+  if (flags & XF_FLAG_V_READY) {
+    st = __uint_as_float((uint32_t)q1);
+    qt = __uint_as_float((uint32_t)(q1 >> 32));
+    return;
+  }
   st = 0.f;
   qt = 0.f;
-  if ((flags & XF_FLAG_V_READY) && (K & 7) == 0) {
-    const float* vp = reinterpret_cast<const float*>(xf_row(t, slot) + 32);
-    for (int k = 0; k < K; k += 8) {
-      float v[8];
-      xf_ld8_l1(vp + k, v);
-#pragma unroll
-      for (int e = 0; e < 8; ++e) { st += v[e]; qt = __fadd_rn(qt, __fmul_rn(v[e], v[e])); }
-    }
-  } else if (flags & XF_FLAG_V_READY) {
-    const float* vp = reinterpret_cast<const float*>(xf_row(t, slot) + 32);
-    for (int k = 0; k < K; k += VEC) {
-      float v[VEC];
-      xf_ldv_step<VEC>(vp + k, v);
-#pragma unroll
-      for (int e = 0; e < VEC; ++e) { st += v[e]; qt = __fadd_rn(qt, __fmul_rn(v[e], v[e])); }
-    }
-  } else {
-    for (int k = 0; k < K; ++k) {
-      const float v = xf_v_init(t, key, (uint32_t)k);
-      st += v;
-      qt = __fadd_rn(qt, __fmul_rn(v, v));
-    }
-  }
+  for (int k = 0; k < t.K; ++k) xf_fm_sums(xf_v_init(t, key, (uint32_t)k), st, qt);
+}
+
+template <bool ADMIT, bool STAMP>
+__device__ __forceinline__ bool xf_fm_look(const XfTableView& t, uint64_t key, uint64_t& s, uint32_t& i, uint64_t& q0,
+                                           uint64_t& q1, uint64_t& q2, uint64_t& q3, uint32_t& slot, bool& created,
+                                           const XfAdmitView& adm, bool& rejected, const XfStampView& sv) {
+  if (q0 == key) { slot = (uint32_t)s; return true; }
+  if (q0 == XF_EMPTY_KEY) {
+    if (ADMIT && !xf_admit(adm, key)) {
+      rejected = adm.mode != XF_ADM_NEVER;
+      return true;
+    }
+    const unsigned long long old =
+        atomicCAS(reinterpret_cast<unsigned long long*>(xf_row(t, s)), (unsigned long long)XF_EMPTY_KEY, (unsigned long long)key);
+    if (old == XF_EMPTY_KEY || old == key) {
+      if (old == XF_EMPTY_KEY) {
+        if (STAMP && sv.stamp != nullptr) sv.stamp[s] = sv.now;
+        created = true;
+      }
+      q0 = key; q1 = q2 = q3 = 0ull;
+      slot = (uint32_t)s;
+      return true;
+    }
+  }
+  if (++i == XF_MAX_PROBE) { *t.error = 1; return true; }
+  s = xf_probe_slot(t, key, i);
+  return false;
 }
 
 template <bool FM, int VEC, bool ADMIT, bool STAMP, bool WEIGHT>
@@ -61,10 +63,10 @@
   const int K = t.K;
   const int NC = (FM && log2nc >= 0) ? (1 << log2nc) : 0;
   double* c_acc = reinterpret_cast<double*>(xf_smem);
-  uint32_t* c_tag = reinterpret_cast<uint32_t*>(xf_smem + (size_t)NC * 24);
+  uint32_t* c_tag = reinterpret_cast<uint32_t*>(xf_smem + (size_t)NC * 16);
   if (NC) {
     for (int e = threadIdx.x; e < NC; e += blockDim.x) c_tag[e] = XF_NO_SLOT;
-    for (int e = threadIdx.x; e < NC * 3; e += blockDim.x) c_acc[e] = 0.0;
+    for (int e = threadIdx.x; e < NC * 2; e += blockDim.x) c_acc[e] = 0.0;
     __syncthreads();
   }
 
@@ -89,26 +91,51 @@
       const bool v0 = j0 < end, v1 = j1 < end;
       const uint64_t k0 = v0 ? __ldcs(keys + j0) : 0ull;
       const uint64_t k1 = v1 ? __ldcs(keys + j1) : 0ull;
-      const uint64_t p0 = xf_home_slot(t, k0), p1 = xf_home_slot(t, k1);
-      XfHead h0, h1;
-      h0.key = h1.key = XF_EMPTY_KEY;
-      if (v0) h0 = FM ? xf_load_head_l1(xf_row(t, p0)) : xf_load_head(xf_row(t, p0));
-      if (v1) h1 = FM ? xf_load_head_l1(xf_row(t, p1)) : xf_load_head(xf_row(t, p1));
+      uint64_t p0 = xf_home_slot(t, k0), p1 = xf_home_slot(t, k1);
       uint32_t s0 = XF_NO_SLOT, s1 = XF_NO_SLOT;
       bool r0 = false, r1 = false;
-      if (v0) {
-        const int64_t r = xf_probe_from<true, ADMIT, STAMP>(t, k0, p0, h0, &adm, &r0, &sv);
-        if (r >= 0) { s0 = (uint32_t)r; wsum += h0.w; }
-      }
-      if (v1) {
-        const int64_t r = xf_probe_from<true, ADMIT, STAMP>(t, k1, p1, h1, &adm, &r1, &sv);
-        if (r >= 0) { s1 = (uint32_t)r; wsum += h1.w; }
-      }
-      if (ADMIT) xf_admit_append(adm, r0, k0, r1, k1);
       if (FM) {
+        uint64_t a0, a1, a2, a3, b0, b1, b2, b3;
+        xf_ld32_pair<true>(v0 ? xf_row(t, p0) : nullptr, a0, a1, a2, a3);
+        xf_ld32_pair<true>(v1 ? xf_row(t, p1) : nullptr, b0, b1, b2, b3);
+        uint32_t i0 = 0, i1 = 0;
+        bool u0 = v0, u1 = v1;
+        for (;;) {
+          bool c0 = false, c1 = false;
+          if (u0) u0 = !xf_fm_look<ADMIT, STAMP>(t, k0, p0, i0, a0, a1, a2, a3, s0, c0, adm, r0, sv);
+          if (u1) u1 = !xf_fm_look<ADMIT, STAMP>(t, k1, p1, i1, b0, b1, b2, b3, s1, c1, adm, r1, sv);
+          const unsigned created = __popc(__ballot_sync(0xffffffffu, c0)) + __popc(__ballot_sync(0xffffffffu, c1));
+          if (created && lane == 0) {
+            atomicAdd(t.size, (unsigned long long)created);
+            if (ADMIT) atomicAdd(adm.admitted, (unsigned long long)created);
+          }
+          if (!__any_sync(0xffffffffu, u0 || u1)) break;
+          uint64_t x0, x1, x2, x3;
+          xf_ld32_pair<true>(u0 ? xf_row(t, p0) : nullptr, x0, x1, x2, x3);
+          if (u0) { a0 = x0; a1 = x1; a2 = x2; a3 = x3; }
+          xf_ld32_pair<true>(u1 ? xf_row(t, p1) : nullptr, x0, x1, x2, x3);
+          if (u1) { b0 = x0; b1 = x1; b2 = x2; b3 = x3; }
+        }
+        if (ADMIT) xf_admit_append(adm, r0, k0, r1, k1);
+        if (s0 != XF_NO_SLOT) wsum += __uint_as_float((uint32_t)a2);
+        if (s1 != XF_NO_SLOT) wsum += __uint_as_float((uint32_t)b2);
         float st, qt;
-        if (s0 != XF_NO_SLOT) { xf_fm_token<VEC>(t, s0, h0.flags, k0, st, qt); ssum += st; qsum += qt; }
-        if (s1 != XF_NO_SLOT) { xf_fm_token<VEC>(t, s1, h1.flags, k1, st, qt); ssum += st; qsum += qt; }
+        if (s0 != XF_NO_SLOT) { xf_fm_token(t, a1, (uint32_t)(a3 >> 32), k0, st, qt); ssum += st; qsum += qt; }
+        if (s1 != XF_NO_SLOT) { xf_fm_token(t, b1, (uint32_t)(b3 >> 32), k1, st, qt); ssum += st; qsum += qt; }
+      } else {
+        XfHead h0, h1;
+        h0.key = h1.key = XF_EMPTY_KEY;
+        if (v0) h0 = xf_load_head(xf_row(t, p0));
+        if (v1) h1 = xf_load_head(xf_row(t, p1));
+        if (v0) {
+          const int64_t r = xf_probe_from<true, ADMIT, STAMP>(t, k0, p0, h0, &adm, &r0, &sv);
+          if (r >= 0) { s0 = (uint32_t)r; wsum += h0.w; }
+        }
+        if (v1) {
+          const int64_t r = xf_probe_from<true, ADMIT, STAMP>(t, k1, p1, h1, &adm, &r1, &sv);
+          if (r >= 0) { s1 = (uint32_t)r; wsum += h1.w; }
+        }
+        if (ADMIT) xf_admit_append(adm, r0, k0, r1, k1);
       }
 #pragma unroll
       for (int c = 0; c < XF_CACHED_CHUNKS; ++c)
@@ -133,12 +160,7 @@
     if (WEIGHT) loss = __fmul_rn(__ldg(wv.e + row), loss);
     abs_acc += fabsf(loss);
 
-    float gw_c = loss;
-    if (FM) {
-      gw_c = 0.f;
-      for (int k = 0; k < K; ++k) gw_c += loss;
-    }
-    const double gw_d = (double)gw_c;
+    const double gw_d = (double)loss;
     for (int ch = 0; ch < chunks; ++ch) {
       const uint32_t j0 = beg + (uint32_t)ch * 64u + (uint32_t)lane;
       const uint32_t j1 = j0 + 32u;
@@ -160,33 +182,37 @@
       const double ld = (double)loss, ad = (double)loss * (double)S;
       double old0 = 0.0, old1 = 0.0;
       bool cached0 = false, cached1 = false;
-      if (NC) {
-        if (lead0) {
-          const uint32_t e = (s0 * 2654435761u) >> (32 - log2nc);
-          const uint32_t prev = atomicCAS(c_tag + e, XF_NO_SLOT, s0);
-          if (prev == XF_NO_SLOT || prev == s0) {
-            cached0 = true;
-            atomicAdd(c_acc + 3 * e, gw_d * c0);
-            atomicAdd(c_acc + 3 * e + 1, ld * c0);
-            atomicAdd(c_acc + 3 * e + 2, ad * c0);
+      if (FM) {
+        const double l0 = __dadd_rn(ld * c0, 0.0), l1 = __dadd_rn(ld * c1, 0.0);
+        if (NC) {
+          if (lead0) {
+            const uint32_t e = (s0 * 2654435761u) >> (32 - log2nc);
+            const uint32_t prev = atomicCAS(c_tag + e, XF_NO_SLOT, s0);
+            if (prev == XF_NO_SLOT || prev == s0) {
+              cached0 = true;
+              atomicAdd(c_acc + 2 * e, l0);
+              atomicAdd(c_acc + 2 * e + 1, ad * c0);
+            }
+          }
+          if (lead1) {
+            const uint32_t e = (s1 * 2654435761u) >> (32 - log2nc);
+            const uint32_t prev = atomicCAS(c_tag + e, XF_NO_SLOT, s1);
+            if (prev == XF_NO_SLOT || prev == s1) {
+              cached1 = true;
+              atomicAdd(c_acc + 2 * e, l1);
+              atomicAdd(c_acc + 2 * e + 1, ad * c1);
+            }
           }
         }
-        if (lead1) {
-          const uint32_t e = (s1 * 2654435761u) >> (32 - log2nc);
-          const uint32_t prev = atomicCAS(c_tag + e, XF_NO_SLOT, s1);
-          if (prev == XF_NO_SLOT || prev == s1) {
-            cached1 = true;
-            atomicAdd(c_acc + 3 * e, gw_d * c1);
-            atomicAdd(c_acc + 3 * e + 1, ld * c1);
-            atomicAdd(c_acc + 3 * e + 2, ad * c1);
-          }
-        }
-      }
-      if (lead0 && !cached0) old0 = atomicAdd(xf_row_g(xf_row(t, s0)), gw_d * c0);
-      if (lead1 && !cached1) old1 = atomicAdd(xf_row_g(xf_row(t, s1)), gw_d * c1);
-      if (FM) {
-        if (lead0 && !cached0) { double* a = xf_row_acc(xf_row(t, s0), K); atomicAdd(a, ld * c0); atomicAdd(a + 1, ad * c0); }
-        if (lead1 && !cached1) { double* a = xf_row_acc(xf_row(t, s1), K); atomicAdd(a, ld * c1); atomicAdd(a + 1, ad * c1); }
+        double* a0 = (lead0 && !cached0) ? xf_row_acc(xf_row(t, s0), K) : nullptr;
+        double* a1 = (lead1 && !cached1) ? xf_row_acc(xf_row(t, s1), K) : nullptr;
+        if (a0) old0 = atomicAdd(a0, l0);
+        if (a1) old1 = atomicAdd(a1, l1);
+        if (a0) atomicAdd(a0 + 1, ad * c0);
+        if (a1) atomicAdd(a1 + 1, ad * c1);
+      } else {
+        if (lead0) old0 = atomicAdd(xf_row_g(xf_row(t, s0)), gw_d * c0);
+        if (lead1) old1 = atomicAdd(xf_row_g(xf_row(t, s1)), gw_d * c1);
       }
       const bool f0 = lead0 && !cached0 && (unsigned long long)__double_as_longlong(old0) == XF_NEG_ZERO_BITS64;
       const bool f1 = lead1 && !cached1 && (unsigned long long)__double_as_longlong(old1) == XF_NEG_ZERO_BITS64;
@@ -200,12 +226,10 @@
       const uint32_t s = c_tag[e];
       uint32_t rec = XF_NO_SLOT;
       if (s != XF_NO_SLOT) {
-        uint8_t* rowp = xf_row(t, s);
-        const double old = atomicAdd(xf_row_g(rowp), c_acc[3 * e]);
+        double* a = xf_row_acc(xf_row(t, s), K);
+        const double old = atomicAdd(a, c_acc[2 * e]);
         if ((unsigned long long)__double_as_longlong(old) == XF_NEG_ZERO_BITS64) rec = s;
-        double* a = xf_row_acc(rowp, K);
-        atomicAdd(a, c_acc[3 * e + 1]);
-        atomicAdd(a + 1, c_acc[3 * e + 2]);
+        atomicAdd(a + 1, c_acc[2 * e + 1]);
       }
       touched[touched_base + (uint32_t)blockIdx.x * (uint32_t)NC + (uint32_t)e] = rec;
     }
@@ -248,7 +272,7 @@
   const int block = 256;
   const int grid = xf_grid_for((uint64_t)B * 32, block, 8);
   const int lg = xf_step_cache_log2(t.K);
-  const size_t smem = lg >= 0 ? ((size_t)1 << lg) * 28 : 0;
+  const size_t smem = lg >= 0 ? ((size_t)1 << lg) * 20 : 0;
 #define XF_STEP_ARGS t, row_ptr, keys, labels, B, mode, touched, loss_out, pctr_out, abs_loss_sum, lg, nnz, a, sv, wv
 #define XF_STEP_LAUNCH_W(A, S, W)                                                             \
   if (t.K == 0) {                                                                             \
diff --git a/xflow_b200/csrc/table.cuh b/xflow_b200/csrc/table.cuh
--- a/xflow_b200/csrc/table.cuh
+++ b/xflow_b200/csrc/table.cuh
@@ -171,16 +171,23 @@
   asm volatile("ld.global.ca.v2.u64 {%0,%1}, [%4];\n\tld.global.ca.v2.u64 {%2,%3}, [%4+16];"
                : "=l"(q0), "=l"(q1), "=l"(q2), "=l"(q3) : "l"(p));
 }
+template <bool L1 = false>
 __device__ __forceinline__ void xf_ld32_pair(const uint8_t* mine, uint64_t& q0, uint64_t& q1, uint64_t& q2, uint64_t& q3) {
   const uint32_t odd = threadIdx.x & 1u;
   const uint8_t* other = (const uint8_t*)__shfl_xor_sync(0xffffffffu, (unsigned long long)mine, 1);
   const uint8_t* r0 = odd ? other : mine;
   const uint8_t* r1 = odd ? mine : other;
   uint64_t x0 = 0, x1 = 0, y0 = 0, y1 = 0;
-  asm volatile("{\n .reg .pred p0, p1;\n setp.ne.u64 p0, %4, 0;\n setp.ne.u64 p1, %5, 0;\n"
-               " @p0 ld.global.cg.v2.u64 {%0,%1}, [%6];\n @p1 ld.global.cg.v2.u64 {%2,%3}, [%7];\n}"
-               : "+l"(x0), "+l"(x1), "+l"(y0), "+l"(y1)
-               : "l"(r0), "l"(r1), "l"(r0 + 16 * odd), "l"(r1 + 16 * odd));
+  if (L1)
+    asm volatile("{\n .reg .pred p0, p1;\n setp.ne.u64 p0, %4, 0;\n setp.ne.u64 p1, %5, 0;\n"
+                 " @p0 ld.global.ca.v2.u64 {%0,%1}, [%6];\n @p1 ld.global.ca.v2.u64 {%2,%3}, [%7];\n}"
+                 : "+l"(x0), "+l"(x1), "+l"(y0), "+l"(y1)
+                 : "l"(r0), "l"(r1), "l"(r0 + 16 * odd), "l"(r1 + 16 * odd));
+  else
+    asm volatile("{\n .reg .pred p0, p1;\n setp.ne.u64 p0, %4, 0;\n setp.ne.u64 p1, %5, 0;\n"
+                 " @p0 ld.global.cg.v2.u64 {%0,%1}, [%6];\n @p1 ld.global.cg.v2.u64 {%2,%3}, [%7];\n}"
+                 : "+l"(x0), "+l"(x1), "+l"(y0), "+l"(y1)
+                 : "l"(r0), "l"(r1), "l"(r0 + 16 * odd), "l"(r1 + 16 * odd));
   const uint64_t m0 = odd ? y0 : x0, m1 = odd ? y1 : x1;
   const uint64_t t0 = __shfl_xor_sync(0xffffffffu, odd ? x0 : y0, 1);
   const uint64_t t1 = __shfl_xor_sync(0xffffffffu, odd ? x1 : y1, 1);
@@ -217,15 +224,6 @@
   h.z = __uint_as_float((uint32_t)q3);
   h.flags = (uint32_t)(q3 >> 32);
   return h;
-}
-
-__device__ __forceinline__ void xf_ld8_l1(const float* p, float (&o)[8]) {
-  uint64_t q0, q1, q2, q3;
-  xf_ld32_ca(p, q0, q1, q2, q3);
-  o[0] = __uint_as_float((uint32_t)q0); o[1] = __uint_as_float((uint32_t)(q0 >> 32));
-  o[2] = __uint_as_float((uint32_t)q1); o[3] = __uint_as_float((uint32_t)(q1 >> 32));
-  o[4] = __uint_as_float((uint32_t)q2); o[5] = __uint_as_float((uint32_t)(q2 >> 32));
-  o[6] = __uint_as_float((uint32_t)q3); o[7] = __uint_as_float((uint32_t)(q3 >> 32));
 }
 
 __device__ __forceinline__ void xf_store_head(uint8_t* row, const XfHead& h) {
@@ -458,6 +456,15 @@
   return false;
 }
 
+__device__ __forceinline__ bool xf_fm_plain(const XfTableView& t) { return t.K > 0 && !t.canon; }
+__device__ __forceinline__ void xf_fm_sums(float v, float& S, float& Q) {
+  S = __fadd_rn(S, v);
+  Q = __fadd_rn(Q, __fmul_rn(v, v));
+}
+__device__ __forceinline__ uint64_t xf_sq_word(float S, float Q) {
+  return (uint64_t)__float_as_uint(S) | ((uint64_t)__float_as_uint(Q) << 32);
+}
+
 __device__ __forceinline__ float xf_warp_sum(float v) {
 #pragma unroll
   for (int o = 16; o > 0; o >>= 1) v += __shfl_xor_sync(0xffffffffu, v, o);
```

Result: no change. 83.62 million (median of 6 runs) (-0.0%).
